# zhuye98/ICL

Measured on AMD Instinct MI355X. Metric: 3D volumes/sec/node (fwd+bwd, 96^3 patch), higher is better.
Workload: dtype f32; 1 GPU; 3D U-Net ICL BraTS-shape synthetic 96x96x96, num_classes=2, batch=2 per GPU (1 labeled + 1 unlabeled), full ICL step incl. SGD; global_batch=2, parallelism=dp1, launch=hipGraph replay

## Files before the change

### icl_amd/_lib.py

```python
from __future__ import annotations

import ctypes
import os
from ctypes import c_char_p, c_float, c_int, c_int64, c_void_p

import torch

_HERE = os.path.dirname(os.path.abspath(__file__))
DEFAULT_LIB = os.path.join(_HERE, "libicl_hip.so")

_lib = None
_lib_path = None
_host_pointers_ok = False

P, I, L, F = c_void_p, c_int, c_int64, c_float

_SIGNATURES = {
    "icl_abi_version": (c_int, []),
    "icl_last_error": (c_char_p, []),
    "icl_last_kernel_name": (c_char_p, []),
    "icl_conv3d_packed_elems": (c_int64, [I, I, I, I]),
    "icl_conv3d_pack_weights": (c_int, [P, P, I, I, I, I, P]),
    "icl_conv3d_pack_weights_both": (c_int, [P, P, P, I, I, I, P]),
    "icl_conv3d_pack_weights_multi": (c_int, [P, P, P, P, P, P, I, P]),
    "icl_conv3d_fwd_ws_bytes": (c_int64, [I, I, I, I, I, I, I]),
    "icl_conv3d_fwd": (c_int, [P, P, P, P, P, I, I, I, I, I, I, I, L, L, P]),
    "icl_scalar_combine": (c_int, [P, P, I, I, P, P]),
    "icl_conv3d_split_ws_bytes": (c_int64, [I, I]),
    "icl_conv3d_split_weights_multi": (c_int, [P, P, P, P, I, P]),
    "icl_conv3d_fwd_presplit": (c_int, [P, P, P, P, I, I, I, I, I, I, L, L, P]),
    "icl_conv3d_fwd_presplit_ws_bytes": (c_int64, [I, I, I, I, I, I]),
    "icl_conv3d_fwd_presplit_ws": (c_int, [P, P, P, P, P, I, I, I, I, I, I, L, L, P]),
    "icl_conv3d_fwd_stats_slots": (c_int, [I, I, I, I, I, I]),
    "icl_conv3d_fwd_presplit_stats": (c_int, [P, P, P, P, P, I, I, I, I, I, I, L, L, P]),
    "icl_norm_fwd_given_stats": (c_int, [P, P, P, P, P, P, P, P, P, I, I, L, I, I, F, F, P, I, P]),
    "icl_conv3d_wgrad_ws_bytes": (c_int64, [I, I, I, I]),
    "icl_conv3d_wgrad": (c_int, [P, P, P, P, P, I, I, I, I, I, I, I, L, L, P]),
    "icl_conv3d_wgrad_slabs": (c_int, [P, P, P, I, I, I, I, I, I, I, L, L, P, P]),
    "icl_conv3d_wgrad_reduce_multi": (c_int, [P, P, P, P, P, P, I, P]),
    "icl_norm_ws_bytes": (c_int64, [I, I, L]),
    "icl_norm_fwd": (c_int, [P, P, P, P, P, P, P, P, I, I, L, I, I, I, F, F, P, P]),
    "icl_norm_bwd": (c_int, [P, P, P, P, P, P, P, P, P, I, I, L, I, I, I, P, P]),
    "icl_norm_res_fwd": (c_int, [P, P, P, P, P, P, P, P, P, I, I, L, I, I, I, F, F, P, P]),
    "icl_norm_res_bwd": (c_int, [P, P, P, P, P, P, P, P, P, P, P, I, I, L, I, I, I, P, P]),
    "icl_rstd_from_var": (c_int, [P, P, I, F, P]),
    "icl_norm_finalize_stats": (c_int, [P, I, I, I, F, P, P, P, P]),
    "icl_norm_apply": (c_int, [P, P, P, I, I, L, P]),
    "icl_maxpool2_fwd_norm": (c_int, [P, P, P, P, L, I, I, I, I, P]),
    "icl_upsample2x_concat_norm": (c_int, [P, P, P, P, P, I, I, I, I, I, I, P]),
    "icl_conv1x1_dropout_norm": (c_int, [P, P, P, P, P, I, I, I, L, I, I, ctypes.c_uint32, F, P, P]),
    "icl_conv1x1_wgrad_dropout_norm": (c_int, [P, P, P, P, P, P, I, I, I, L, L, ctypes.c_uint32, F, P, P]),
    "icl_maxpool2_fwd": (c_int, [P, P, P, L, I, I, I, I, P]),
    "icl_maxpool2_bwd": (c_int, [P, P, P, L, I, I, I, I, P]),
    "icl_maxpool2_bwd_add": (c_int, [P, P, P, P, I, I, I, I, I, I, L, P]),
    "icl_trilinear_fwd": (c_int, [P, P, I, I, I, I, I, I, I, I, L, I, P]),
    "icl_trilinear_bwd_ws_bytes": (c_int64, [I, I, I, I, I, I, I, I]),
    "icl_trilinear_bwd": (c_int, [P, P, P, I, I, I, I, I, I, I, I, L, I, P]),
    "icl_copy_rows": (c_int, [P, P, L, L, L, L, P]),
    "icl_concat2": (c_int, [P, L, P, L, P, P]),
    "icl_dwconv3_fwd": (c_int, [P, P, P, I, I, I, I, I, I, P]),
    "icl_dwconv3_wgrad_ws_bytes": (c_int64, [I, I, I, I, I]),
    "icl_dwconv3_wgrad": (c_int, [P, P, P, P, I, I, I, I, I, P]),
    "icl_conv1x1_small": (c_int, [P, P, P, P, I, I, I, L, I, I, P]),
    "icl_conv1x1_dropout": (c_int, [P, P, P, P, I, I, I, L, I, I, I, ctypes.c_uint32, F, P, P]),
    "icl_conv1x1_wgrad_dropout": (c_int, [P, P, P, P, P, I, I, I, L, L, ctypes.c_uint32, F, P, P]),
    "icl_dropout": (c_int, [P, P, L, ctypes.c_uint32, F, P, P]),
    "icl_drop_path": (c_int, [P, P, L, L, ctypes.c_uint32, F, P, P]),
    "icl_drop_path_add": (c_int, [P, P, P, L, L, ctypes.c_uint32, F, P, P]),
    "icl_loss_fwd": (c_int, [P, P, P, P, P, P, I, I, L, I, I, P]),
    "icl_window_attn_bias_elems": (c_int64, [I, I]),
    "icl_depth_to_space2": (c_int, [P, P, I, I, I, I, I, L, P]),
    "icl_space_to_depth2": (c_int, [P, P, I, I, I, I, I, L, P]),
    "icl_colsum_multi": (c_int, [P, P, P, P, I, P]),
    "icl_gather_rows": (c_int, [P, P, P, L, L, L, I, P]),
    "icl_gather_rows_sum2": (c_int, [P, P, P, L, L, L, I, P]),
    "icl_im2col3": (c_int, [P, P, I, I, I, I, I, P]),
    "icl_im2col3_planes": (c_int, [P, P, I, I, I, I, I, P]),
    "icl_conv3d_cin1_fwd": (c_int, [P, P, P, P, I, I, I, I, I, L, L, P]),
    "icl_conv3d_cin1_wgrad_ws_bytes": (c_int64, [I, I, I]),
    "icl_conv3d_cin1_wgrad": (c_int, [P, P, P, P, I, I, I, I, I, L, L, P]),
    "icl_col2im3": (c_int, [P, P, I, I, I, I, I, P]),
    "icl_linear_ws_bytes": (c_int64, [L, I, I, I]),
    "icl_linear_fwd": (c_int, [P, P, P, P, P, L, I, I, I, P]),
    "icl_linear_dgrad": (c_int, [P, P, P, P, L, I, I, P]),
    "icl_linear_bwd_small": (c_int, [P, P, P, P, P, P, L, I, I, P]),
    "icl_linear_wgrad_small": (c_int, [P, P, P, P, L, I, I, P]),
    "icl_linear_dgrad_sgd": (c_int, [P, P, P, P, P, P, L, I, I, F, F, F, I, P, P]),
    "icl_gemm_ws_bytes": (c_int64, [L, I, I, I]),
    "icl_gemm": (c_int, [P, P, P, P, P, L, I, I, L, L, L, I, I, I, I, L, L, L, P]),
    "icl_linear_wgrad_ws_bytes": (c_int64, [L, I, I]),
    "icl_linear_wgrad": (c_int, [P, P, P, P, P, L, I, I, P]),
    "icl_conv1x1_wgrad_ws_bytes": (c_int64, [I, L, I, I]),
    "icl_conv1x1_wgrad": (c_int, [P, P, P, P, P, I, I, I, L, L, L, P]),
    "icl_relpos_bias_fwd": (c_int, [P, P, P, I, I, I, P]),
    "icl_window_attn_fwd": (c_int, [P, P, P, P, P, I, I, I, I, I, F, P]),
    "icl_window_attn_bwd": (c_int, [P, P, P, P, P, P, P, P, I, I, I, I, I, F, P]),
    "icl_window_attn_bwd_chunks": (c_int, [I, I, I, I, I]),
    "icl_relpos_bias_bwd_sum": (c_int, [P, I, P, P, P, L, I, I, P]),
    "icl_layernorm_fwd": (c_int, [P, P, P, P, P, P, L, I, F, P]),
    "icl_layernorm_bwd_ws_bytes": (c_int64, [L, I]),
    "icl_layernorm_bwd": (c_int, [P, P, P, P, P, P, P, P, P, L, I, P]),
    "icl_gelu_fwd": (c_int, [P, P, L, P]),
    "icl_gelu_bwd": (c_int, [P, P, P, L, P]),
    "icl_attn_fwd": (c_int, [P, P, P, P, P, I, I, I, I, I, F, P]),
    "icl_attn_bwd": (c_int, [P, P, P, P, P, P, P, P, P, I, I, I, I, I, F, P]),
    "icl_attn_bwd_ws_bytes": (c_int64, [I, I, I, I, I]),
    "icl_attn_bwd_ws": (c_int, [P, P, P, P, P, P, P, P, P, P, I, I, I, I, I, F, P]),
    "icl_crop_rotflip": (c_int, [P, P, P, I, P, P, I, I, I, P]),
    "icl_sgd_step": (c_int, [P, P, P, L, F, F, F, I, P, P]),
    "icl_sgd_step_factored": (c_int, [P, P, P, P, I, I, I, F, F, F, I, P, P]),
    "icl_sgd_step_factored_narrow": (c_int, [P, P, P, P, I, I, I, F, F, F, I, P, I, P]),
    "icl_sgd_factored_split_ws_bytes": (c_int64, [I, I, I]),
    "icl_sgd_step_factored_split": (c_int, [P, P, P, P, P, I, I, I, F, F, F, I, P, P]),
    "icl_sgd_step_multi": (c_int, [P, P, P, P, I, F, F, F, I, P, P]),
    "icl_loss_bwd": (c_int, [P, P, P, P, P, P, P, P, I, I, L, I, I, P]),
    "icl_loss_fwd_multi": (c_int, [P, I, P]),
    "icl_loss_bwd_multi": (c_int, [P, I, P]),
    "icl_qchain_stage": (c_int, [P, P]),
    "icl_qchain_wgrad": (c_int, [P, P, P, P, P, P, P, P, I, P]),
    "icl_seg_metrics_ws_bytes": (c_int64, [I, I, I, I]),
    "icl_seg_metrics": (c_int, [P, I, P, I, I, I, I, I, I, P, P, P]),
}

EXPORTS = tuple(_SIGNATURES)


def _load(path: str):
    if not os.path.exists(path):
        raise RuntimeError(
            f"icl_amd: HIP library {path} not found — build it with `python -m icl_amd.build` "
            "(hipcc --offload-arch=gfx950). There is no CPU fallback.")
    lib = ctypes.CDLL(path)
    for name, (res, args) in _SIGNATURES.items():
        fn = getattr(lib, name)
        fn.restype = res
        fn.argtypes = args
    return lib


def lib():
    global _lib, _lib_path
    if _lib is None:
        _lib_path = os.environ.get("ICL_HIP_LIB", DEFAULT_LIB)
        _lib = _load(_lib_path)
    return _lib


def lib_path():
    lib()
    return _lib_path


def host_pointers_ok() -> bool:
    return _host_pointers_ok


def _use_library_for_tests(path: str | None, host_pointers: bool = True):
    global _lib, _lib_path, _host_pointers_ok
    if path is None:
        _lib, _lib_path, _host_pointers_ok = None, None, False
        return
    _lib, _lib_path, _host_pointers_ok = _load(path), path, host_pointers


def check(rc: int, what: str = ""):
    if rc != 0:
        msg = lib().icl_last_error()
        raise RuntimeError(f"icl_hip {what} failed ({rc}): {msg.decode() if msg else ''}")
```

### icl_amd/csrc/icl_abi.inc

```

#include "kernels/common.h"
#include "kernels/norm.h"
#include "kernels/pool_resize.h"
#include "kernels/reduce.h"
#include "kernels/conv_mfma.h"
#include "kernels/conv_mfma_static.h"
#include "kernels/conv_mfma_flat.h"
#include "kernels/conv_bf16x3.h"
#include "kernels/conv_bf16x3_ws.h"
#include "kernels/conv_wgrad_tr.h"
#include "kernels/conv_wgrad_zs.h"
#include "kernels/conv_cin1.h"
#include "kernels/misc.h"
#include "kernels/loss.h"
#include "kernels/optim.h"
#include "kernels/winattn.h"
#include "kernels/linear_wgrad.h"
#include "kernels/token.h"
#include "kernels/gemm.h"
#include "kernels/datafeed.h"
#include "kernels/qchain.h"
#include "kernels/metrics.h"

#ifdef ICL_TWO_UNITS
// ... 992 lines not shown
int icl_conv3d_wgrad_slabs(const float* x, const float* gy, void* ws, int n, int cin, int cout, int d, int h, int w, int ks,
                           int64_t x_bstride, int64_t gy_bstride, int32_t* nslabs, void* stream) {
  if (!x || !gy || !ws || !nslabs || n < 1 || cin < 1 || cout < 1 || (ks != 1 && ks != 3)) return fail(-1, "conv3d_wgrad_slabs: bad argument");
  int ns = 0;
  const int rc = ks == 3 ? conv_wgrad_launch<3>(x, gy, (float*)ws, n, cin, cout, d, h, w, x_bstride, gy_bstride, &ns, (hipStream_t)stream)
                         : conv_wgrad_launch<1>(x, gy, (float*)ws, n, cin, cout, d, h, w, x_bstride, gy_bstride, &ns, (hipStream_t)stream);
  *nslabs = ns;
  return rc;
}

int icl_conv3d_wgrad_reduce_multi(const void* const* ws, void* const* gw, const int32_t* cout, const int32_t* cin, const int32_t* ks,
                                  const int32_t* nslabs, int count, void* stream) {
  if (!ws || !gw || !cout || !cin || !ks || !nslabs || count < 1) return fail(-1, "conv3d_wgrad_reduce_multi: bad argument");
  for (int base = 0; base < count; base += icl::kReduceMulti) {
    icl::ReduceMulti m{};
    const int k = count - base < icl::kReduceMulti ? count - base : icl::kReduceMulti;
    long most = 1;
    for (int i = 0; i < k; ++i) {
      const int j = base + i;
      if (!ws[j] || !gw[j] || cout[j] < 1 || cin[j] < 1 || (ks[j] != 1 && ks[j] != 3) || nslabs[j] < 1)
        return fail(-1, "conv3d_wgrad_reduce_multi: bad job %d", j);
      const long pe = icl_conv3d_packed_elems(cout[j], cin[j], ks[j], 0);
      m.gwp[i] = (const float*)ws[j]; m.gw[i] = (float*)gw[j];
      m.cout[i] = cout[j]; m.cin[i] = cin[j]; m.taps[i] = ks[j] * ks[j] * ks[j]; m.nslabs[i] = nslabs[j];
      m.tall[i] = wgrad_reduce_tall(nslabs[j], pe) ? 1 : 0;
      const long blocks = m.tall[i] ? cdivl(pe, 16) : cdivl(pe, 64);
      if (blocks > most) most = blocks;
    }
    ICL_LAUNCH(icl::reduce_unpack_wgrad_multi_kernel, dim3((unsigned)(most < 1024 ? most : 1024), k), dim3(256), 0, (hipStream_t)stream, m);
    const int rc = check_launch("reduce_unpack_wgrad_multi");
    if (rc) return rc;
  }
  return 0;
}

int icl_conv3d_wgrad(const float* x, const float* gy, float* gw, float* gbias, void* ws, int n, int cin, int cout, int d,
                     int h, int w, int ks, int64_t x_bstride, int64_t gy_bstride, void* stream) {
  if (!x || !gy || !gw || !ws || n < 1 || cin < 1 || cout < 1 || (ks != 1 && ks != 3)) return fail(-1, "conv3d_wgrad: bad argument");
  hipStream_t s = (hipStream_t)stream;
  float* gwp = (float*)ws;
  int nslabs = 0;
  int rc = ks == 3 ? conv_wgrad_launch<3>(x, gy, gwp, n, cin, cout, d, h, w, x_bstride, gy_bstride, &nslabs, s)
                   : conv_wgrad_launch<1>(x, gy, gwp, n, cin, cout, d, h, w, x_bstride, gy_bstride, &nslabs, s);
  if (rc) return rc;
  const int T = ks * ks * ks;
  const long total = (long)cout * cin * T;
  (void)total;
  const long pe_all = icl_conv3d_packed_elems(cout, cin, ks, 0);
  if (wgrad_reduce_tall(nslabs, pe_all))
    ICL_LAUNCH(icl::reduce_unpack_wgrad_tall_kernel, dim3((unsigned)cdivl(pe_all, 16)), dim3(256), 0, s, (const float*)gwp, gw, cout, cin, T,
               round_up(cin, 4), round_up(cout, 16), nslabs);
  else
    ICL_LAUNCH(icl::reduce_unpack_wgrad_kernel, dim3(grid_for(pe_all, 64)), dim3(256), 0, s, (const float*)gwp, gw, cout, cin, T,
               round_up(cin, 4), round_up(cout, 16), nslabs);
  rc = check_launch("reduce_unpack_wgrad");
  if (rc) return rc;
  if (gbias) {
    const long S = (long)d * h * w;
    long chunks = cdivl(S, 16384);
    if (chunks > 16) chunks = 16;
    const long clen = round_up(cdivl(S, chunks), 4);
    chunks = cdivl(S, clen);
    float* part = (float*)ws;
    dim3 grid((unsigned)chunks, cout, n);
    ICL_LAUNCH(icl::channel_sum_kernel, grid, dim3(256), 0, s, gy, part, S, (long)gy_bstride, clen);
    rc = check_launch("channel_sum");
    if (rc) return rc;
    const void* g[1] = {part};
    void* out[1] = {gbias};
    const int32_t rr[1] = {(int32_t)(n * chunks)}, cc[1] = {cout};
    rc = icl_colsum_multi(g, out, rr, cc, 1, stream);
  }
  return rc;
}

int64_t icl_norm_ws_bytes(int n, int c, int64_t s) {
  const int64_t nch = (s + icl::kNormChunk - 1) / icl::kNormChunk;
  return ((int64_t)n * c * nch * 3 + (int64_t)n * c * 2 + 64) * 4;
}

namespace {
inline bool norm_one_launch() {
  constexpr int on = 1;
  return on != 0;
}
}

int icl_norm_fwd(const float* x, float* y, float* mean, float* rstd, const float* gamma, const float* beta,
                 float* running_mean, float* running_var, int n, int c, int64_t s, int mode, int use_batch_stats,
                 int act, float eps, float momentum, void* ws, void* stream) {
  return icl_norm_res_fwd(x, nullptr, y, mean, rstd, gamma, beta, running_mean, running_var, n, c, s, mode, use_batch_stats, act,
                          eps, momentum, ws, stream);
}

int icl_norm_res_fwd(const float* x, const float* res, float* y, float* mean, float* rstd, const float* gamma, const float* beta,
                     float* running_mean, float* running_var, int n, int c, int64_t s, int mode, int use_batch_stats,
                     int act, float eps, float momentum, void* ws, void* stream) {
  if (!x || !y || !mean || !rstd || n < 1 || c < 1 || s < 1) return fail(-1, "norm_fwd: bad argument");
  hipStream_t st = (hipStream_t)stream;
  const int R = n * c;
  const int nch = (int)((s + icl::kNormChunk - 1) / icl::kNormChunk);
  const float* part = nullptr;
  const int inline_stats = (use_batch_stats && mode == 0 && nch == 1 && !running_mean && norm_one_launch()) ? 1 : 0;
  if (use_batch_stats && !inline_stats) {
    if (!ws) return fail(-1, "norm_fwd: workspace required");
    ICL_LAUNCH(icl::rowstats_partial_kernel, dim3(nch, R), dim3(icl::kNormThreads), 0, st, x, (float*)ws, (long)s, nch);
    if (int rc = check_launch("rowstats_partial")) return rc;
    part = (const float*)ws;
  }
  ICL_LAUNCH(icl::norm_act_fwd_kernel, dim3(nch, R), dim3(icl::kNormThreads), 0, st, x, y, mean, rstd, gamma, beta, (long)s, c, mode, act, res,
             part, R, nch, eps, running_mean, running_var, momentum, inline_stats);
  return check_launch("norm_act_fwd");
}

int icl_norm_fwd_given_stats(const float* x, const float* res, float* y, float* mean, float* rstd, const float* gamma, const float* beta,
                             float* running_mean, float* running_var, int n, int c, int64_t s, int mode, int act, float eps,
                             float momentum, const float* part, int nslots, void* stream) {
  if (!x || !y || !mean || !rstd || !part || n < 1 || c < 1 || s < 1 || nslots < 1) return fail(-1, "norm_fwd_given_stats: bad argument");
  const int R = n * c;
  const int nch = (int)((s + icl::kNormChunk - 1) / icl::kNormChunk);
  ICL_LAUNCH(icl::norm_act_fwd_kernel, dim3(nch, R), dim3(icl::kNormThreads), 0, (hipStream_t)stream, x, y, mean, rstd, gamma, beta, (long)s, c,
             mode, act, res, part, R, nslots, eps, running_mean, running_var, momentum, 0);
  return check_launch("norm_act_fwd");
}

int icl_norm_bwd(const float* gy, const float* x, const float* mean, const float* rstd, const float* gamma,
                 const float* beta, float* gx, float* dgamma, float* dbeta, int n, int c, int64_t s, int mode,
                 int use_batch_stats, int act, void* ws, void* stream) {
  return icl_norm_res_bwd(gy, x, nullptr, mean, rstd, gamma, beta, gx, nullptr, dgamma, dbeta, n, c, s, mode, use_batch_stats, act,
                          ws, stream);
}

int icl_norm_res_bwd(const float* gy, const float* x, const float* res, const float* mean, const float* rstd, const float* gamma,
                     const float* beta, float* gx, float* gres, float* dgamma, float* dbeta, int n, int c, int64_t s, int mode,
                     int use_batch_stats, int act, void* ws, void* stream) {
  if (!gy || !x || !mean || !rstd || !gx || !ws || n < 1 || c < 1 || s < 1) return fail(-1, "norm_bwd: bad argument");
  hipStream_t st = (hipStream_t)stream;
  const int R = n * c;
  const int nch = (int)((s + icl::kNormChunk - 1) / icl::kNormChunk);
  float* part = (float*)ws;
  if (mode == 0 && nch == 1 && norm_one_launch()) {
    part = nullptr;
  } else {
    ICL_LAUNCH(icl::norm_act_bwd_partial_kernel, dim3(nch, R), dim3(icl::kNormThreads), 0, st, gy, x, mean, rstd, gamma, beta, part,
               (long)s, c, nch, mode, act, res);
    if (int rc = check_launch("norm_bwd_partial")) return rc;
  }
  const float inv_count = 1.0f / (float)((mode ? (int64_t)n : 1) * s);
  ICL_LAUNCH(icl::norm_act_bwd_apply_kernel, dim3(nch, R), dim3(icl::kNormThreads), 0, st, gy, x, mean, rstd, gamma, beta,
             (const float*)part, gx, (long)s, c, mode, act, inv_count, use_batch_stats, res, gres, R, nch, dgamma, dbeta);
  return check_launch("norm_bwd_apply");
}

int icl_rstd_from_var(const float* var, float* rstd, int c, float eps, void* stream) {
  if (!var || !rstd || c < 1) return fail(-1, "rstd_from_var: bad argument");
  ICL_LAUNCH(icl::rstd_from_var_kernel, dim3((c + 63) / 64), dim3(64), 0, (hipStream_t)stream, var, rstd, c, eps);
  return check_launch("rstd_from_var");
}

namespace {
int maxpool2_fwd_run(const float* x, const float* ss, float* y, uint8_t* idx, int64_t nc, int dout, int hout, int wout, int pool_depth,
                     hipStream_t st, const char* what) {
  const long total = nc * dout * hout * wout;
  const char* e_x2 = getenv("ICL_MAXPOOL_BWD_X2");
  if ((wout & 1) == 0 && aligned16(x) && ((uintptr_t)y & 7) == 0 && (e_x2 ? atoi(e_x2) : 1)) {
    ICL_LAUNCH(icl::maxpool2_fwd_x2_kernel, dim3(grid_for(total / 2, 256)), dim3(256), 0, st, x, y, idx, (long)nc, dout, hout, wout, pool_depth, ss);
  } else {
    ICL_LAUNCH(icl::maxpool2_fwd_kernel, dim3(grid_for(total, 256)), dim3(256), 0, st, x, y, idx, (long)nc, dout, hout, wout, pool_depth, ss);
  }
  return check_launch(what);
}
}

int icl_maxpool2_fwd(const float* x, float* y, uint8_t* idx, int64_t nc, int dout, int hout, int wout, int pool_depth, void* stream) {
  if (!x || !y || !idx || nc < 1 || dout < 1 || hout < 1 || wout < 1 || (pool_depth != 1 && pool_depth != 2)) return fail(-1, "maxpool2_fwd: bad argument");
  return maxpool2_fwd_run(x, nullptr, y, idx, nc, dout, hout, wout, pool_depth, (hipStream_t)stream, "maxpool2_fwd");
}

int icl_norm_finalize_stats(const float* part, int n, int c, int nslots, float eps, float* mean, float* rstd, float* ss, void* stream) {
  if (!part || !mean || !rstd || !ss || n < 1 || c < 1 || nslots < 1) return fail(-1, "norm_finalize_stats: bad argument");
  ICL_LAUNCH(icl::norm_finalize_stats_kernel, dim3(n * c), dim3(64), 0, (hipStream_t)stream, part, n * c, c, nslots, eps, mean, rstd, ss);
  return check_launch("norm_finalize_stats");
}

int icl_norm_apply(const float* x, const float* ss, float* y, int n, int c, int64_t s, void* stream) {
  if (!x || !ss || !y || n < 1 || c < 1 || s < 4 || (s & 3) || !aligned16(x) || !aligned16(y)) return fail(-1, "norm_apply: bad argument (s %% 4 == 0)");
  ICL_LAUNCH(icl::copy_rows_norm_kernel, dim3(grid_for((long)n * c * (s >> 2), 256, 1 << 16)), dim3(256), 0, (hipStream_t)stream, x, y, n, c, (long)s,
             (long)c * s, ss);
  return check_launch("norm_apply");
}

int icl_maxpool2_fwd_norm(const float* x, const float* ss, float* y, uint8_t* idx, int64_t nc, int dout, int hout, int wout, int pool_depth,
                          void* stream) {
  if (!x || !ss || !y || !idx || nc < 1 || dout < 1 || hout < 1 || wout < 1 || (pool_depth != 1 && pool_depth != 2))
    return fail(-1, "maxpool2_fwd_norm: bad argument");
  return maxpool2_fwd_run(x, ss, y, idx, nc, dout, hout, wout, pool_depth, (hipStream_t)stream, "maxpool2_fwd_norm");
}

int icl_upsample2x_concat_norm(const float* skip, const float* skip_ss, const float* deep, const float* deep_ss, float* out, int n, int cs,
                               int cd, int d, int h, int w, void* stream) {
  if (!skip || !deep || !out || n < 1 || cs < 1 || cd < 1 || d < 2 || h < 2 || w < 4 || (d & 1) || (h & 1) || (w & 3))
    return fail(-1, "upsample2x_concat_norm: bad argument (even depth / height, width a multiple of 4)");
  if (!aligned16(skip) || !aligned16(deep) || !aligned16(out)) return fail(-1, "upsample2x_concat_norm: 16-byte alignment");
  hipStream_t st = (hipStream_t)stream;
  const long s = (long)d * h * w, obs = (long)(cs + cd) * s;
  if (skip_ss) {
    ICL_LAUNCH(icl::copy_rows_norm_kernel, dim3(grid_for((long)n * cs * (s >> 2), 256, 1 << 16)), dim3(256), 0, st, skip, out, n, cs, s, obs, skip_ss);
  } else {
    ICL_LAUNCH(icl::copy_rows_kernel, dim3(grid_for((long)n * cs * s, 256)), dim3(256), 0, st, skip, out, (long)n, (long)cs * s, (long)cs * s, obs);
  }
  if (int rc = check_launch("upsample2x_concat_norm: skip")) return rc;
  const long total = (long)n * cd * s;
  const int di = d / 2, hi = h / 2, wi = w / 2;
  if (wi % 4 == 0)
    ICL_LAUNCH(icl::upsample2x_fwd_x4_kernel, dim3(grid_for(total / 32, 256, 1 << 16)), dim3(256), 0, st, deep, out + (long)cs * s, n, cd, di, hi, wi, obs,
               deep_ss);
  else
    ICL_LAUNCH(icl::upsample2x_fwd_kernel, dim3(grid_for(total / 16, 256, 1 << 16)), dim3(256), 0, st, deep, out + (long)cs * s, n, cd, di, hi, wi, obs,
               deep_ss);
  return check_launch("upsample2x_concat_norm: deep");
}

int icl_maxpool2_bwd(const float* gy, const uint8_t* idx, float* gx, int64_t nc, int dout, int hout, int wout, int pool_depth, void* stream) {
  if (!gy || !gx || !idx || nc < 1 || dout < 1 || hout < 1 || wout < 1 || (pool_depth != 1 && pool_depth != 2)) return fail(-1, "maxpool2_bwd: bad argument");
  const long total = nc * dout * hout * wout;
  ICL_LAUNCH(icl::maxpool2_bwd_kernel, dim3(grid_for(total, 256)), dim3(256), 0, (hipStream_t)stream, gy, idx, gx, (long)nc, dout, hout, wout,
             pool_depth);
  return check_launch("maxpool2_bwd");
}

int icl_maxpool2_bwd_add(const float* gy, const uint8_t* idx, const float* add, float* gx, int n, int c, int dout, int hout, int wout,
                         int pool_depth, int64_t add_bstride, void* stream) {
  if (!gy || !gx || !idx || !add || n < 1 || c < 1 || dout < 1 || hout < 1 || wout < 1 || (pool_depth != 1 && pool_depth != 2) || (add_bstride & 1) ||
      ((uintptr_t)add & 7))
    return fail(-1, "maxpool2_bwd_add: bad argument");
  const long total = (long)n * c * dout * hout * wout;
  const char* e_x2 = getenv("ICL_MAXPOOL_BWD_X2");
  if ((wout & 1) == 0 && aligned16(add) && aligned16(gx) && ((uintptr_t)gy & 7) == 0 && (add_bstride & 3) == 0 && (e_x2 ? atoi(e_x2) : 1)) {
    ICL_LAUNCH(icl::maxpool2_bwd_add_x2_kernel, dim3(grid_for(total / 2, 256)), dim3(256), 0, (hipStream_t)stream, gy, idx, add, gx, (long)n * c, c,
               dout, hout, wout, pool_depth, (long)add_bstride);
    return check_launch("maxpool2_bwd_add_x2");
  }
  ICL_LAUNCH(icl::maxpool2_bwd_add_kernel, dim3(grid_for(total, 256)), dim3(256), 0, (hipStream_t)stream, gy, idx, add, gx, (long)n * c, c, dout,
             hout, wout, pool_depth, (long)add_bstride);
  return check_launch("maxpool2_bwd_add");
}

namespace {
inline float resize_scale(int in, int out, int align) {
  if (align) return out > 1 ? (float)(in - 1) / (float)(out - 1) : 0.f;
  return (float)in / (float)out;
}
}

int icl_trilinear_fwd(const float* x, float* y, int n, int c, int di, int hi, int wi, int dout, int hout, int wout,
                      int64_t y_bstride, int align_corners, void* stream) {
  if (!x || !y || n < 1 || c < 1 || di < 1 || hi < 1 || wi < 1 || dout < 1 || hout < 1 || wout < 1) return fail(-1, "trilinear_fwd: bad argument");
  const long total = (long)n * c * dout * hout * wout;
  const float rz = resize_scale(di, dout, align_corners), ry = resize_scale(hi, hout, align_corners), rx = resize_scale(wi, wout, align_corners);
  if (!align_corners && dout == 2 * di && hout == 2 * hi && wout == 2 * wi && wi % 2 == 0 && y_bstride % 4 == 0 && aligned16(y) &&
      total / 16 < (1L << 31)) {
    constexpr int x4 = 1;
    if (x4 && wi % 4 == 0 && aligned16(x))
      ICL_LAUNCH(icl::upsample2x_fwd_x4_kernel, dim3(grid_for(total / 32, 256, 1 << 16)), dim3(256), 0, (hipStream_t)stream, x, y, n, c, di, hi,
                 wi, (long)y_bstride, (const float*)nullptr);
    else
      ICL_LAUNCH(icl::upsample2x_fwd_kernel, dim3(grid_for(total / 16, 256, 1 << 16)), dim3(256), 0, (hipStream_t)stream, x, y, n, c, di, hi, wi,
                 (long)y_bstride, (const float*)nullptr);
  } else if (wout % 4 == 0 && y_bstride % 4 == 0 && aligned16(y) && total / 4 < (1L << 31)) {
    ICL_LAUNCH(icl::trilinear_fwd_quad_kernel, dim3(grid_for(total / 4, 256, 1 << 16)), dim3(256), 0, (hipStream_t)stream, x, y, n, c, di, hi,
               wi, dout, hout, wout, rz, ry, rx, (long)y_bstride, align_corners);
  } else {
    ICL_LAUNCH(icl::trilinear_fwd_kernel, dim3(grid_for(total, 256)), dim3(256), 0, (hipStream_t)stream, x, y, n, c, di, hi, wi, dout, hout,
               wout, rz, ry, rx, (long)y_bstride, align_corners);
  }
  return check_launch("trilinear_fwd");
}

int64_t icl_trilinear_bwd_ws_bytes(int n, int c, int di, int hi, int wi, int dout, int hout, int wout) {
  (void)di;
  return ((int64_t)n * c * dout * hout * wi + (int64_t)n * c * dout * hi * wi) * 4;
}

int icl_trilinear_bwd(const float* gy, float* gx, void* ws, int n, int c, int di, int hi, int wi, int dout, int hout, int wout,
                      int64_t gy_bstride, int align_corners, void* stream) {
  if (!gy || !gx || !ws || n < 1 || c < 1 || di < 1 || hi < 1 || wi < 1 || dout < 1 || hout < 1 || wout < 1) return fail(-1, "trilinear_bwd: bad argument");
  hipStream_t st = (hipStream_t)stream;
  const int al = align_corners;
  const float rz = resize_scale(di, dout, al), ry = resize_scale(hi, hout, al), rx = resize_scale(wi, wout, al);
  float* t1 = (float*)ws;
  float* t2 = t1 + (size_t)n * c * dout * hout * wi;
  int rc;
  if (!al && dout == 2 * di && hout == 2 * hi && wout == 2 * wi && wi % 4 == 0 && gy_bstride % 4 == 0 && aligned16(gy) && aligned16(gx) &&
      (long)n * c * di * hi * wi / 4 < (1L << 31)) {
    ICL_LAUNCH(icl::upsample2x_bwd_kernel, dim3(grid_for((long)n * c * ((di + icl::kUpSeg - 1) / icl::kUpSeg) * hi * wi / 4, 256, 1 << 16)),
               dim3(256), 0, st, gy, gx, n, c, di, hi,
               wi, (long)gy_bstride);
    return check_launch("upsample2x_bwd");
  }
  auto axis = [&](const float* src, float* dst, long rows, int li, int lo, long inner, float rs, long sbs, const char* what) -> int {
    const long total = (long)n * rows * li * inner;
    const bool small = total / 4 < (1L << 31) && rows < (1L << 31);
    if (small && inner % 4 == 0 && sbs % 4 == 0 && aligned16(src) && aligned16(dst)) {
      ICL_LAUNCH(icl::resize_bwd_axis_t4_kernel, dim3(grid_for(total / 4, 256, 1 << 16)), dim3(256), 0, st, src, dst, n, (unsigned)rows, li, lo,
                 (unsigned)(inner / 4), rs, sbs, al);
    } else if (inner == 1 && lo >= 4 * li && lo % 4 == 0 && lo <= 1024 && sbs % 4 == 0 && aligned16(src) && rows * li >= 4096) {
      const long nrows = (long)n * rows;
      ICL_LAUNCH(icl::resize_bwd_axis_x_lds_kernel, dim3((unsigned)cdivl(nrows, icl::kRbxRows)), dim3(256),
                 (size_t)icl::kRbxRows * (lo + 4) * 4, st, src, dst, n, rows, li, lo, rs, sbs, al);
    } else if (small && inner == 1 && li % 4 == 0 && aligned16(dst)) {
      ICL_LAUNCH(icl::resize_bwd_axis_i4_kernel, dim3(grid_for(total / 4, 256, 1 << 16)), dim3(256), 0, st, src, dst, n, (unsigned)rows, li, lo,
                 rs, sbs, al);
    } else {
      ICL_LAUNCH(icl::resize_bwd_axis_kernel, dim3(grid_for(total, 256)), dim3(256), 0, st, src, dst, n, rows, li, lo, inner, rs, sbs, al);
    }
    return check_launch(what);
  };
  if ((rc = axis(gy, t1, (long)c * dout * hout, wi, wout, 1L, rx, (long)gy_bstride, "resize_bwd_x"))) return rc;
  if ((rc = axis(t1, t2, (long)c * dout, hi, hout, (long)wi, ry, (long)c * dout * hout * wi, "resize_bwd_y"))) return rc;
  if ((rc = axis(t2, gx, (long)c, di, dout, (long)hi * wi, rz, (long)c * dout * hi * wi, "resize_bwd_z"))) return rc;
  return 0;
}

int icl_copy_rows(const float* src, float* dst, int64_t rows, int64_t row_elems, int64_t src_stride, int64_t dst_stride,
                  void* stream) {
  if (!src || !dst || rows < 1 || row_elems < 1) return fail(-1, "copy_rows: bad argument");
  ICL_LAUNCH(icl::copy_rows_kernel, dim3(grid_for(rows * row_elems, 256)), dim3(256), 0, (hipStream_t)stream, src, dst, (long)rows,
             (long)row_elems, (long)src_stride, (long)dst_stride);
  return check_launch("copy_rows");
}

int icl_concat2(const float* a, int64_t na, const float* b, int64_t nb, float* out, void* stream) {
  if (!out || na < 0 || nb < 0 || na + nb < 4 || (na & 3) || (nb & 3) || (!a && !b)) return fail(-1, "concat2: bad argument (float counts are multiples of 4)");
  if ((a && !aligned16(a)) || (b && !aligned16(b)) || !aligned16(out)) return fail(-1, "concat2: 16-byte alignment");
  ICL_LAUNCH(icl::concat2_kernel, dim3(grid_for((na + nb) >> 2, 256)), dim3(256), 0, (hipStream_t)stream, a, (long)na, b, (long)nb, out);
  return check_launch("concat2");
}

int icl_depth_to_space2(const float* yt, float* out, int n, int d, int h, int w, int cout, int64_t out_bstride, void* stream) {
  if (!yt || !out || n < 1 || d < 1 || h < 1 || w < 1 || cout < 1) return fail(-1, "depth_to_space2: bad argument");
  const size_t lds = (size_t)w * (cout * 8 + 2) * 4;
  if (lds > (size_t)kMaxDynLdsBig) return fail(-1, "depth_to_space2: token row does not fit LDS (w * cout too large)");
  if (lds > (size_t)kMaxDynLds) ICL_SET_MAX_DYN_LDS(icl::depth_to_space2_kernel, kMaxDynLdsBig);
  ICL_LAUNCH(icl::depth_to_space2_kernel, dim3(h, d, n), dim3(256), lds, (hipStream_t)stream, yt, out, d, h, w, cout, (long)out_bstride);
  return check_launch("depth_to_space2");
}

int icl_space_to_depth2(const float* g, float* gt, int n, int d, int h, int w, int cout, int64_t g_bstride, void* stream) {
  if (!g || !gt || n < 1 || d < 1 || h < 1 || w < 1 || cout < 1) return fail(-1, "space_to_depth2: bad argument");
  const size_t lds = (size_t)w * (cout * 8 + 2) * 4;
  if (lds > (size_t)kMaxDynLdsBig) return fail(-1, "space_to_depth2: token row does not fit LDS (w * cout too large)");
  if (lds > (size_t)kMaxDynLds) ICL_SET_MAX_DYN_LDS(icl::space_to_depth2_kernel, kMaxDynLdsBig);
  ICL_LAUNCH(icl::space_to_depth2_kernel, dim3(h, d, n), dim3(256), lds, (hipStream_t)stream, g, gt, d, h, w, cout, (long)g_bstride);
  return check_launch("space_to_depth2");
}

int icl_dwconv3_fwd(const float* x, const float* w, float* y, int n, int c, int d, int h, int wd, int flip, void* stream) {
  if (!x || !w || !y || n < 1 || c < 1 || d < 1 || h < 1 || wd < 1) return fail(-1, "dwconv3_fwd: bad argument");
  const long total = (long)n * c * d * h * wd;
  ICL_LAUNCH(icl::dwconv3_fwd_kernel, dim3(grid_for(total, 256)), dim3(256), 0, (hipStream_t)stream, x, w, y, (long)n * c, c, d, h, wd, flip);
  return check_launch("dwconv3_fwd");
}

static long dwconv3_wgrad_chunks(long total) {
  long chunks = cdivl(total, 1024);
  return chunks > 512 ? 512 : chunks;
}

int64_t icl_dwconv3_wgrad_ws_bytes(int n, int c, int d, int h, int wd) {
  return dwconv3_wgrad_chunks((long)n * d * h * wd) * c * 27 * 4;
}

int icl_dwconv3_wgrad(const float* x, const float* gy, float* gw, void* ws, int n, int c, int d, int h, int wd, void* stream) {
  if (!x || !gy || !gw || !ws || n < 1 || c < 1 || d < 1 || h < 1 || wd < 1) return fail(-1, "dwconv3_wgrad: bad argument");
  hipStream_t s = (hipStream_t)stream;
  const long total = (long)n * d * h * wd;
  const long chunks = dwconv3_wgrad_chunks(total);
  const long chunk = cdivl(total, chunks);
  ICL_LAUNCH(icl::dwconv3_wgrad_kernel, dim3((unsigned)chunks, c), dim3(256), 0, s, x, gy, (float*)ws, n, c, d, h, wd, chunk);
  if (int rc = check_launch("dwconv3_wgrad")) return rc;
  ICL_LAUNCH(icl::dwconv3_wgrad_reduce_kernel, dim3((unsigned)cdivl((long)c * 27, 16)), dim3(256), 0, s, (const float*)ws, gw, c * 27, (int)chunks);
  return check_launch("dwconv3_wgrad_reduce");
}

namespace {
icl::DropSpec drop_spec(int mode, uint32_t seed, float p, const uint32_t* seed_dev) {
  icl::DropSpec d{};
  d.mode = mode;
  d.seed = (unsigned)seed;
  d.thresh = (unsigned)((double)p * 4294967296.0);
  d.scale = 1.0f / (1.0f - p);
  d.seed_dev = (const unsigned*)seed_dev;
  return d;
}

int conv1x1_small_run(const float* x, const float* w, const float* bias, float* y, int n, int cin, int cout, int64_t s, int w_ostride,
                      int w_istride, const icl::DropSpec& dr, hipStream_t st) {
  if ((long)n * s >= 65536) {
// ... 278 lines not shown
  if (c >= 1024 && c <= 256 * 64 && longrow) {
    if (c <= 256 * 16) ICL_LAUNCH((icl::layernorm_bwd_longrow_kernel<16>), dim3((unsigned)rows), dim3(256), 0, st, gy, x, gamma, mean, rstd, gx, c);
    else if (c <= 256 * 32) ICL_LAUNCH((icl::layernorm_bwd_longrow_kernel<32>), dim3((unsigned)rows), dim3(256), 0, st, gy, x, gamma, mean, rstd, gx, c);
    else ICL_LAUNCH((icl::layernorm_bwd_longrow_kernel<64>), dim3((unsigned)rows), dim3(256), 0, st, gy, x, gamma, mean, rstd, gx, c);
  } else if (c >= 1024) {
    ICL_LAUNCH((icl::layernorm_bwd_kernel<true>), dim3((unsigned)rows), dim3(256), 0, st, gy, x, gamma, mean, rstd, gx, (long)rows, c);
  } else {
    ICL_LAUNCH((icl::layernorm_bwd_kernel<false>), dim3((unsigned)cdivl(rows, 4)), dim3(256), 0, st, gy, x, gamma, mean, rstd, gx,
               (long)rows, c);
  }
  int rc = check_launch("layernorm_bwd");
  if (rc || !ws) return rc;
  int cols = 256;
  while (cols > c && cols > 16) cols >>= 1;
  if (cols < c && cols < 256) cols <<= 1;
  ICL_LAUNCH(icl::layernorm_wgrad_kernel, dim3((c + cols - 1) / cols, (unsigned)chunks), dim3(256), 0, st, gy, x, mean, rstd, part_g, part_b,
             (long)rows, c, rpb, cols);
  rc = check_launch("layernorm_wgrad");
  if (rc || !dgamma) return rc;
  const void* g[2] = {part_g, part_b};
  void* out[2] = {dgamma, dbeta};
  const int32_t rr[2] = {chunks, chunks}, cc[2] = {c, c};
  return icl_colsum_multi(g, out, rr, cc, 2, stream);
}

int icl_gelu_fwd(const float* x, float* y, int64_t n, void* stream) {
  if (!x || !y || n < 1) return fail(-1, "gelu_fwd: bad argument");
  ICL_LAUNCH(icl::gelu_fwd_kernel, dim3(grid_for(n, 256)), dim3(256), 0, (hipStream_t)stream, x, y, (long)n);
  return check_launch("gelu_fwd");
}

int icl_gelu_bwd(const float* gy, const float* x, float* gx, int64_t n, void* stream) {
  if (!gy || !x || !gx || n < 1) return fail(-1, "gelu_bwd: bad argument");
  ICL_LAUNCH(icl::gelu_bwd_kernel, dim3(grid_for(n, 256)), dim3(256), 0, (hipStream_t)stream, gy, x, gx, (long)n);
  return check_launch("gelu_bwd");
}

int icl_attn_fwd(const float* q, const float* kv, float* logits, float* out, float* stats, int b, int h, int nc, int n, int d,
                 float scale, void* stream) {
  if (!q || !kv || !logits || !out || !stats || b < 1 || h < 1 || nc < 1 || nc > icl::kAttnMaxNc || n < 1 || (d != 8 && d != 16))
    return fail(-1, "attn_fwd: bad argument (nc <= 16, head dim 8 or 16)");
  hipStream_t st = (hipStream_t)stream;
  const dim3 g1((n + 255) / 256, b * h), g2(b * h * nc);
  if (d == 16) {
    ICL_LAUNCH((icl::attn_logits_kernel<16>), g1, dim3(256), 0, st, q, kv, logits, b, h, nc, n, scale);
    ICL_LAUNCH((icl::attn_softmax_pv_kernel<16, 256>), g2, dim3(256), 0, st, (const float*)logits, kv, out, stats, b, h, nc, n);
  } else {
    ICL_LAUNCH((icl::attn_logits_kernel<8>), g1, dim3(256), 0, st, q, kv, logits, b, h, nc, n, scale);
    ICL_LAUNCH((icl::attn_softmax_pv_kernel<8, 256>), g2, dim3(256), 0, st, (const float*)logits, kv, out, stats, b, h, nc, n);
  }
  return check_launch("attn_fwd");
}

int64_t icl_attn_bwd_ws_bytes(int b, int h, int nc, int n, int d) {
  if (b < 1 || h < 1 || nc < 1 || n < 1 || d < 1) return 0;
  return (int64_t)((n + 255) / 256) * b * h * nc * d * 4;
}

int icl_attn_bwd(const float* q, const float* kv, const float* logits, const float* stats, const float* out, const float* gout,
                 const float* glog, float* gq, float* gkv, int b, int h, int nc, int n, int d, float scale, void* stream) {
  return icl_attn_bwd_ws(q, kv, logits, stats, out, gout, glog, gq, gkv, nullptr, b, h, nc, n, d, scale, stream);
}

int icl_attn_bwd_ws(const float* q, const float* kv, const float* logits, const float* stats, const float* out, const float* gout,
                    const float* glog, float* gq, float* gkv, void* ws, int b, int h, int nc, int n, int d, float scale, void* stream) {
  if (!q || !kv || !logits || !stats || !out || !gq || !gkv || b < 1 || h < 1 || nc < 1 || nc > icl::kAttnMaxNc || n < 1 ||
      (d != 8 && d != 16))
    return fail(-1, "attn_bwd: bad argument");
  hipStream_t st = (hipStream_t)stream;
  const dim3 g1((n + 255) / 256, b * h), g2(b * h * nc);
  float* pq = (float*)ws;
  if (d == 16) {
    ICL_LAUNCH((icl::attn_bwd_kv_kernel<16>), g1, dim3(256), 0, st, q, kv, logits, stats, out, gout, glog, gkv, b, h, nc, n, scale, pq);
    if (!pq) ICL_LAUNCH((icl::attn_bwd_q_kernel<16, 256>), g2, dim3(256), 0, st, kv, logits, stats, out, gout, glog, gq, b, h, nc, n, scale);
  } else {
    ICL_LAUNCH((icl::attn_bwd_kv_kernel<8>), g1, dim3(256), 0, st, q, kv, logits, stats, out, gout, glog, gkv, b, h, nc, n, scale, pq);
    if (!pq) ICL_LAUNCH((icl::attn_bwd_q_kernel<8, 256>), g2, dim3(256), 0, st, kv, logits, stats, out, gout, glog, gq, b, h, nc, n, scale);
  }
  if (pq) {
    const int rd = b * h * nc * d;
    ICL_LAUNCH(icl::attn_dq_reduce_kernel, dim3((rd + 255) / 256), dim3(256), 0, st, (const float*)pq, gq, (int)g1.x, rd, scale);
  }
  return check_launch("attn_bwd");
}

int64_t icl_window_attn_bias_elems(int n, int heads) { return icl_window_attn_bias_elems_impl(n, heads); }

static int linear_wgrad_nsplit(int64_t rows, int o, int i) {
  const int ob = (o + icl::kLwB - 1) / icl::kLwB, ib = (i + icl::kLwB - 1) / icl::kLwB;
  long n = rows * (o + i) / ((long)o * i + o);
  const long want = (2048 + ob * ib - 1) / (ob * ib);
  if (n > want) n = want;
  const long steps = (rows + 3) / 4;
  if (n > steps / 8) n = steps / 8;
  if (n < 4) n = 4;
  return (int)((n + 3) / 4 * 4);
}

int64_t icl_linear_wgrad_ws_bytes(int64_t rows, int o, int i) {
  return (int64_t)linear_wgrad_nsplit(rows, o, i) * ((int64_t)o * i + o) * 4;
}

int icl_linear_wgrad(const float* gy, const float* x, float* dw, float* db, void* ws, int64_t rows, int o, int i, void* stream) {
  if (!gy || !x || !dw || !ws || rows < 1 || o < 1 || i < 1) return fail(-1, "linear_wgrad: bad argument");
  hipStream_t st = (hipStream_t)stream;
  const int nsplit = linear_wgrad_nsplit(rows, o, i);
  const int ob = (o + icl::kLwB - 1) / icl::kLwB, ib = (i + icl::kLwB - 1) / icl::kLwB;
  ICL_LAUNCH(icl::linear_wgrad_kernel, dim3(nsplit / 4, ob, ib), dim3(256), 0, st, gy, x, (float*)ws, (long)rows, o, i, nsplit);
  if (int rc = check_launch("linear_wgrad")) return rc;
  const long EW = (long)o * i, E = EW + o;
  ICL_LAUNCH(icl::linear_wgrad_reduce_kernel, dim3((unsigned)cdivl(E, 16)), dim3(256), 0, st, (const float*)ws, dw, db, E, EW, nsplit);
  return check_launch("linear_wgrad_reduce");
}

static bool cin1_geom(icl::Cin1Geom& g, int n, int cout, int d, int h, int w, int64_t xbs, int64_t ybs) {
  if (n < 1 || cout < 1 || cout > 16 || d < 1 || h < 1 || w < 1 || (long)d * h * w * 16 >= (1L << 31)) return false;
  g.N = n; g.Cout = cout; g.D = d; g.H = h; g.W = w; g.nty = (h + icl::kC1Rows - 1) / icl::kC1Rows;
  g.x_bstride = xbs; g.y_bstride = ybs; g.ntiles = n * d * g.nty;
  return (size_t)3 * (icl::kC1Rows + 2) * (w + 2) * 4 <= 64 * 1024;
}
static int cin1_grid(const icl::Cin1Geom& g) { return g.ntiles < 2048 ? g.ntiles : 2048; }
static size_t cin1_lds(const icl::Cin1Geom& g) {
  const size_t halo = (size_t)3 * (icl::kC1Rows + 2) * (g.W + 2) * 4;
  return halo > 2048 * 4 ? halo : 2048 * 4;
}

int icl_conv3d_cin1_fwd(const float* x, const float* w, const float* bias, float* y, int n, int cout, int d, int h, int wd, int64_t x_bstride,
                        int64_t y_bstride, void* stream) {
  icl::Cin1Geom g;
  if (!x || !w || !y || !cin1_geom(g, n, cout, d, h, wd, x_bstride, y_bstride)) return fail(-1, "conv3d_cin1_fwd: bad argument");
  ICL_LAUNCH(icl::conv_cin1_fwd_kernel, dim3(cin1_grid(g)), dim3(icl::kC1Threads), cin1_lds(g), (hipStream_t)stream, x, w, bias, y, g);
  snprintf(g_kernel, sizeof(g_kernel), "conv_cin1_fwd_kernel");
  return check_launch("conv3d_cin1_fwd");
}

int64_t icl_conv3d_cin1_wgrad_ws_bytes(int n, int d, int h) {
  const long tiles = (long)n * d * ((h + icl::kC1Rows - 1) / icl::kC1Rows);
  return (tiles < 2048 ? tiles : 2048) * 512 * 4;
}

int icl_conv3d_cin1_wgrad(const float* x, const float* gy, float* gw, void* ws, int n, int cout, int d, int h, int wd, int64_t x_bstride,
                          int64_t gy_bstride, void* stream) {
  icl::Cin1Geom g;
  if (!x || !gy || !gw || !ws || (wd & 3) || (gy_bstride & 3) || !aligned16(gy) || !cin1_geom(g, n, cout, d, h, wd, x_bstride, gy_bstride))
    return fail(-1, "conv3d_cin1_wgrad: bad argument (W and the sample stride of dY must be multiples of 4, dY 16-byte aligned)");
  const int grid = cin1_grid(g);
  ICL_LAUNCH(icl::conv_cin1_wgrad_kernel, dim3(grid), dim3(icl::kC1Threads), cin1_lds(g), (hipStream_t)stream, x, gy, (float*)ws, g);
  if (int rc = check_launch("conv3d_cin1_wgrad")) return rc;
  ICL_LAUNCH(icl::conv_cin1_wgrad_reduce_kernel, dim3(16), dim3(256), 0, (hipStream_t)stream, (const float*)ws, gw, grid, cout);
  snprintf(g_kernel, sizeof(g_kernel), "conv_cin1_wgrad_kernel");
  return check_launch("conv3d_cin1_wgrad_reduce");
}

int64_t icl_conv1x1_wgrad_ws_bytes(int n, int64_t s, int cin, int cout) { return icl_linear_wgrad_ws_bytes((int64_t)n * s, cout, cin); }

namespace {
int conv1x1_wgrad_run(const float* x, const float* gy, float* gw, float* gbias, void* ws, int n, int cin, int cout, int64_t s,
                      int64_t x_bstride, int64_t gy_bstride, const icl::DropSpec& dr, hipStream_t st) {
  const int nsplit = linear_wgrad_nsplit((int64_t)n * s, cout, cin);
  const int ob = (cout + icl::kLwB - 1) / icl::kLwB, ib = (cin + icl::kLwB - 1) / icl::kLwB;
  ICL_LAUNCH(icl::conv1x1_wgrad_kernel, dim3(nsplit / 4, ob, ib), dim3(256), 0, st, gy, x, (float*)ws, n, (long)s, cout, cin, nsplit,
             (long)gy_bstride, (long)x_bstride, dr);
  if (int rc = check_launch("conv1x1_wgrad")) return rc;
  const long EW = (long)cout * cin, E = EW + cout;
  ICL_LAUNCH(icl::linear_wgrad_reduce_kernel, dim3((unsigned)cdivl(E, 16)), dim3(256), 0, st, (const float*)ws, gw, gbias, E, EW, nsplit);
  return check_launch("conv1x1_wgrad_reduce");
}
}

int icl_conv1x1_wgrad(const float* x, const float* gy, float* gw, float* gbias, void* ws, int n, int cin, int cout, int64_t s,
                      int64_t x_bstride, int64_t gy_bstride, void* stream) {
  if (!x || !gy || !gw || !ws || n < 1 || cin < 1 || cout < 1 || s < 4 || (s & 3) || (x_bstride & 3) || (gy_bstride & 3))
    return fail(-1, "conv1x1_wgrad: bad argument (voxel count and batch strides must be multiples of 4)");
  return conv1x1_wgrad_run(x, gy, gw, gbias, ws, n, cin, cout, s, x_bstride, gy_bstride, icl::DropSpec{}, (hipStream_t)stream);
}

int icl_conv1x1_wgrad_dropout(const float* x, const float* gy, float* gw, float* gbias, void* ws, int n, int cin, int cout, int64_t s,
                              int64_t gy_bstride, uint32_t seed, float p, const uint32_t* seed_dev, void* stream) {
  if (!x || !gy || !gw || !ws || n < 1 || cin < 1 || cout < 1 || s < 4 || (s & 3) || (gy_bstride & 3) || !(p >= 0.f && p < 1.f))
    return fail(-1, "conv1x1_wgrad_dropout: bad argument");
  return conv1x1_wgrad_run(x, gy, gw, gbias, ws, n, cin, cout, s, (int64_t)cin * s, gy_bstride, drop_spec(1, seed, p, seed_dev), (hipStream_t)stream);
}

int icl_conv1x1_wgrad_dropout_norm(const float* x, const float* ss, const float* gy, float* gw, float* gbias, void* ws, int n, int cin, int cout,
                                   int64_t s, int64_t gy_bstride, uint32_t seed, float p, const uint32_t* seed_dev, void* stream) {
  if (!x || !ss || !gy || !gw || !ws || n < 1 || cin < 1 || cout < 1 || s < 4 || (s & 3) || (gy_bstride & 3) || !(p >= 0.f && p < 1.f))
    return fail(-1, "conv1x1_wgrad_dropout_norm: bad argument");
  icl::DropSpec dr = p > 0.f ? drop_spec(1, seed, p, seed_dev) : icl::DropSpec{};
  dr.ss = ss;
  return conv1x1_wgrad_run(x, gy, gw, gbias, ws, n, cin, cout, s, (int64_t)cin * s, gy_bstride, dr, (hipStream_t)stream);
}

int icl_relpos_bias_fwd(const float* table, const int64_t* index, float* bias, int n, int heads, int idx_stride, void* stream) {
  if (!table || !index || !bias || n < 1 || n > idx_stride || heads < 1) return fail(-1, "relpos_bias_fwd: bad argument");
  const int npad = (n + 15) / 16 * 16;
  ICL_LAUNCH(icl::relpos_bias_gather_kernel, dim3(grid_for((long)heads * n * npad, 256)), dim3(256), 0, (hipStream_t)stream, table,
             (const long*)index, bias, n, npad, heads, idx_stride);
  return check_launch("relpos_bias_fwd");
}

int icl_window_attn_fwd(const float* qkv, const float* bias, const int32_t* regions, float* out, float* lse, int b_, int n, int heads,
                        int nw, int head_dim, float scale, void* stream) {
  if (!qkv || !bias || !out || !lse) return fail(-1, "window_attn_fwd: null pointer");
  icl::WinAttnGeom g;
  if (int rc = winattn_geom(g, b_, n, heads, nw, head_dim, scale, "window_attn_fwd")) return rc;
  const int nkb = g.npad / 16;
  hipStream_t st = (hipStream_t)stream;
  const char* e_on = getenv("ICL_WINATTN_ONLINE");
  const int online = e_on ? atoi(e_on) : 1;
  if (head_dim == 16 && ((nkb > 6 && (long)g.B_ * g.heads >= 512 && online == 1) || online == 2)) {
    const size_t lds = ((size_t)2 * g.npad * (16 + 4) + g.npad) * 4;
    ICL_SET_MAX_DYN_LDS((icl::window_attn_fwd_online_kernel<16>), 64 * 1024);
    ICL_LAUNCH((icl::window_attn_fwd_online_kernel<16>), dim3((unsigned)g.B_ * g.heads), dim3(icl::kWaThreads), lds, st, qkv, bias, regions,
               out, lse, g);
    snprintf(g_kernel, sizeof(g_kernel), "window_attn_fwd_online_kernel<16>");
    return check_launch("window_attn_fwd_online");
  }
  if (head_dim == 32) return winattn_fwd_launch<6, 32>(qkv, bias, regions, out, lse, g, st);
  if (nkb > 14) return winattn_fwd_launch<22, 16>(qkv, bias, regions, out, lse, g, st);
  if (nkb > 6) return winattn_fwd_launch<14, 16>(qkv, bias, regions, out, lse, g, st);
  return winattn_fwd_launch<6, 16>(qkv, bias, regions, out, lse, g, st);
}

int icl_window_attn_bwd(const float* qkv, const float* bias, const int32_t* regions, const float* out, const float* lse,
                        const float* dout, float* dqkv, float* dbias, int b_, int n, int heads, int nw, int head_dim, float scale,
                        void* stream) {
  if (!qkv || !bias || !out || !lse || !dout || !dqkv) return fail(-1, "window_attn_bwd: null pointer");
  icl::WinAttnGeom g;
  if (int rc = winattn_geom(g, b_, n, heads, nw, head_dim, scale, "window_attn_bwd")) return rc;
  hipStream_t st = (hipStream_t)stream;
  if (int rc = head_dim == 32 ? winattn_kv_launch<32>(qkv, bias, regions, out, lse, dout, dqkv, g, st)
                              : winattn_kv_launch<16>(qkv, bias, regions, out, lse, dout, dqkv, g, st))
    return rc;
  const int nkb = g.npad / 16;
  if (head_dim == 32) return winattn_q_bias_launch<6, 32>(qkv, bias, regions, out, lse, dout, dqkv, dbias, g, st);
  if (nkb > 14) return winattn_q_bias_launch<22, 16>(qkv, bias, regions, out, lse, dout, dqkv, dbias, g, st);
  if (nkb > 6) return winattn_q_bias_launch<14, 16>(qkv, bias, regions, out, lse, dout, dqkv, dbias, g, st);
  return winattn_q_bias_launch<6, 16>(qkv, bias, regions, out, lse, dout, dqkv, dbias, g, st);
}

int icl_window_attn_bwd_chunks(int b_, int n, int heads, int nw, int head_dim) {
  icl::WinAttnGeom g;
  if (winattn_geom(g, b_, n, heads, nw, head_dim, 1.f, "window_attn_bwd_chunks")) return 0;
  return winattn_bias_chunks(g);
}

int icl_relpos_bias_bwd_sum(float* dbias, int chunks, const int32_t* inv, const int32_t* offs, float* dtable, int64_t table_rows, int n,
                            int heads, void* stream) {
  if (!dbias || !inv || !offs || !dtable || chunks < 1 || n < 1 || heads < 1 || table_rows < 1)
    return fail(-1, "relpos_bias_bwd_sum: bad argument");
  const int npad = (n + 15) / 16 * 16;
  if (chunks > 1) {
    const long slab = (long)heads * n * npad;
    ICL_LAUNCH(icl::relpos_bias_slab_sum_kernel, dim3(grid_for(slab / 4, 256, 1024)), dim3(256), 0, (hipStream_t)stream, dbias,
               slab, chunks);
    if (int rc = check_launch("relpos_bias_slab_sum")) return rc;
  }
  ICL_LAUNCH(icl::relpos_bias_gather_sum_kernel, dim3((unsigned)((table_rows + 3) / 4), heads), dim3(256), 0, (hipStream_t)stream, dbias, inv,
             offs, dtable, (int)table_rows, n, npad, heads, 1);
  return check_launch("relpos_bias_bwd_sum");
}

int icl_sgd_step(float* p, const float* g, float* m, int64_t n, float lr, float momentum, float weight_decay, int first,
                 const float* lr_dev, void* stream) {
  if (!p || !g || !m || n < 1) return fail(-1, "sgd_step: bad argument");
  ICL_LAUNCH(icl::sgd_momentum_kernel, dim3(grid_for((n + 3) / 4, 256, 4096)), dim3(256), 0, (hipStream_t)stream, p, g, m, (long)n, lr,
             momentum, weight_decay, first, lr_dev);
  return check_launch("sgd_step");
}

int64_t icl_sgd_factored_split_ws_bytes(int rows, int n, int k) {
  if (rows < 1 || n < 1 || k < 1) return 0;
  return (int64_t)3 * ((rows + 7) / 8) * ((int64_t)n + k) * 16;
}

int icl_sgd_step_factored_split(float* p, float* m, const float* g, const float* x, void* ws, int rows, int n, int k, float lr,
                                float momentum, float weight_decay, int first, const float* lr_dev, void* stream) {
  if (!p || !m || !g || !x || !ws || rows < 1 || n < 1 || k < 4 || (k & 3) || !aligned16(ws))
    return fail(-1, "sgd_step_factored_split: bad argument (k %% 4 == 0, workspace of icl_sgd_factored_split_ws_bytes)");
  hipStream_t st = (hipStream_t)stream;
  const int mb = (rows + 7) / 8;
  uint4* gs = (uint4*)ws;
  uint4* xs = gs + (size_t)3 * mb * n;
  ICL_LAUNCH(icl::factor_split_kernel, dim3(grid_for((long)mb * ((long)n + k), 256, 2048)), dim3(256), 0, st, g, x, gs, xs, rows, n, k);
  int rc = check_launch("factor_split");
  if (rc) return rc;
  const size_t lds = (size_t)icl::kSfLdsFloats * 4;
  ICL_SET_MAX_DYN_LDS(icl::sgd_factored_split_kernel, kMaxDynLdsBig);
  ICL_LAUNCH(icl::sgd_factored_split_kernel, dim3((k + icl::kSfCols - 1) / icl::kSfCols, (n + icl::kSfRows - 1) / icl::kSfRows), dim3(256), lds,
             st, p, m, (const uint4*)gs, (const uint4*)xs, rows, n, k, lr, momentum, weight_decay, first, lr_dev);
  return check_launch("sgd_step_factored_split");
}

int icl_sgd_step_factored(float* p, float* m, const float* g, const float* x, int rows, int n, int k, float lr, float momentum,
                          float weight_decay, int first, const float* lr_dev, void* stream) {
  if (!p || !m || !g || !x || rows < 1 || n < 1 || k < 4 || (k & 3)) return fail(-1, "sgd_step_factored: bad argument (k %% 4 == 0)");
  if (rows <= 16) {
    constexpr int variant = 2;
    const dim3 grid((k + icl::kSvCols - 1) / icl::kSvCols, (n + icl::kSvRows - 1) / icl::kSvRows);
    if (variant == 2) {
      ICL_LAUNCH(icl::sgd_factored_small_kernel<2>, grid, dim3(256), 0, (hipStream_t)stream, p, m, g, x, rows, n, k, lr, momentum, weight_decay,
                 first, lr_dev);
    } else if (variant == 1) {
      ICL_LAUNCH(icl::sgd_factored_small_kernel<1>, grid, dim3(256), 0, (hipStream_t)stream, p, m, g, x, rows, n, k, lr, momentum, weight_decay,
                 first, lr_dev);
    } else {
// ... 317 lines not shown
```

### icl_amd/csrc/kernels/conv_cin1.h

```cpp
#pragma once

namespace icl {

constexpr int kC1Rows = 8, kC1Threads = 256;

struct Cin1Geom {
  int N, Cout, D, H, W, nty;
  long x_bstride, y_bstride;
  int ntiles;
};

__device__ __forceinline__ void c1_stage_halo(float* xs, const float* __restrict__ x, const Cin1Geom& g, int n, int z, int y0) {
  const int PW = g.W + 2, PR = kC1Rows + 2;
  const long HW = (long)g.H * g.W;
  const float* xb = x + (long)n * g.x_bstride;
  for (int it = threadIdx.x; it < 3 * PR * PW; it += kC1Threads) {
    const int px = it % PW, row = it / PW, py = row % PR, pz = row / PR;
    const int gz = z - 1 + pz, gy = y0 - 1 + py, gx = px - 1;
    float v = 0.f;
    if ((unsigned)gz < (unsigned)g.D && (unsigned)gy < (unsigned)g.H && (unsigned)gx < (unsigned)g.W) v = xb[gz * HW + (long)gy * g.W + gx];
    xs[it] = v;
  }
}

__global__ __launch_bounds__(kC1Threads) void conv_cin1_wgrad_kernel(const float* __restrict__ x, const float* __restrict__ gy,
                                                                     float* __restrict__ part, Cin1Geom g) {
  ICL_DYN_LDS(float, xs);
  const int lane = threadIdx.x & 63, wid = threadIdx.x >> 6, lr = lane & 15, lg = lane >> 4;
  const int PW = g.W + 2, PR = kC1Rows + 2;
  const long HW = (long)g.H * g.W, DHW = g.D * HW;
  int toff[2];
  bool tok[2];
#pragma unroll
  for (int tb = 0; tb < 2; ++tb) {
    const int tap = 16 * tb + lr;
    tok[tb] = tap < 27;
    const int t = tok[tb] ? tap : 0;
    toff[tb] = (t / 9) * PR * PW + ((t / 3) % 3) * PW + t % 3;
  }
  f32x4 acc[2] = {f32x4{0.f, 0.f, 0.f, 0.f}, f32x4{0.f, 0.f, 0.f, 0.f}};
  for (int tile = blockIdx.x; tile < g.ntiles; tile += gridDim.x) {
    const int n = tile / (g.D * g.nty), rem = tile % (g.D * g.nty), z = rem / g.nty, y0 = (rem % g.nty) * kC1Rows;
    __syncthreads();
    c1_stage_halo(xs, x, g, n, z, y0);
    __syncthreads();
    const float* gb = gy + (long)n * g.y_bstride + (long)lr * DHW + (long)z * HW;
    for (int rr = 0; rr < 2; ++rr) {
      const int ty = 2 * wid + rr, yy = y0 + ty;
      if (yy >= g.H) break;
      const float* grow = gb + (long)yy * g.W;
      const float* xrow = xs + (ty * PW);
      for (int x0 = 0; x0 < g.W; x0 += 16) {
        const int xl = x0 + 4 * lg;
        float4 a = make_float4(0.f, 0.f, 0.f, 0.f);
        if (lr < g.Cout && xl < g.W) a = *reinterpret_cast<const float4*>(grow + xl);
        const float av[4] = {a.x, a.y, a.z, a.w};
        const bool in = xl < g.W;
#pragma unroll
        for (int j = 0; j < 4; ++j) {
#pragma unroll
          for (int tb = 0; tb < 2; ++tb) {
            const float b = (tok[tb] && in) ? xrow[toff[tb] + xl + j] : 0.f;
            acc[tb] = icl_mfma_16x16x4(av[j], b, acc[tb]);
          }
        }
      }
    }
  }
  __syncthreads();
  float* red = xs;
#pragma unroll
  for (int tb = 0; tb < 2; ++tb)
#pragma unroll
    for (int r = 0; r < 4; ++r) red[((wid * 2 + tb) * 4 + r) * 64 + lane] = acc[tb][r];
  __syncthreads();
  if (wid == 0) {
#pragma unroll
    for (int tb = 0; tb < 2; ++tb)
#pragma unroll
      for (int r = 0; r < 4; ++r) {
        float s = 0.f;
#pragma unroll
        for (int w = 0; w < 4; ++w) s += red[((w * 2 + tb) * 4 + r) * 64 + lane];
        part[(long)blockIdx.x * 512 + (4 * lg + r) * 32 + 16 * tb + lr] = s;
      }
  }
}

__global__ __launch_bounds__(256) void conv_cin1_wgrad_reduce_kernel(const float* __restrict__ part, float* __restrict__ gw, int nparts, int cout) {
  __shared__ float sl[8][32];
  const int o = threadIdx.x & 31, slice = threadIdx.x >> 5, e = blockIdx.x * 32 + o;
  float s = 0.f;
#pragma unroll 8
  for (int p = slice; p < nparts; p += 8) s += part[(long)p * 512 + e];
  sl[slice][o] = s;
  __syncthreads();
  if (slice == 0) {
    float t = 0.f;
#pragma unroll
    for (int k = 0; k < 8; ++k) t += sl[k][o];
    const int co = e >> 5, tap = e & 31;
    if (co < cout && tap < 27) gw[co * 27 + tap] = t;
  }
}

__global__ __launch_bounds__(kC1Threads) void conv_cin1_fwd_kernel(const float* __restrict__ x, const float* __restrict__ w,
                                                                   const float* __restrict__ bias, float* __restrict__ y, Cin1Geom g) {
  ICL_DYN_LDS(float, xs);
  const int lane = threadIdx.x & 63, wid = threadIdx.x >> 6, lr = lane & 15, lg = lane >> 4;
  const int PW = g.W + 2, PR = kC1Rows + 2;
  const long HW = (long)g.H * g.W, DHW = g.D * HW;
  float wa[7];
  int toff[7];
#pragma unroll
  for (int s = 0; s < 7; ++s) {
    const int tap = 4 * s + lg;
    wa[s] = (tap < 27 && lr < g.Cout) ? w[lr * 27 + tap] : 0.f;
    const int t = tap < 27 ? tap : 0;
    toff[s] = (t / 9) * PR * PW + ((t / 3) % 3) * PW + t % 3;
  }
  float bv[4];
#pragma unroll
  for (int r = 0; r < 4; ++r) bv[r] = (bias && 4 * lg + r < g.Cout) ? bias[4 * lg + r] : 0.f;
  for (int tile = blockIdx.x; tile < g.ntiles; tile += gridDim.x) {
    const int n = tile / (g.D * g.nty), rem = tile % (g.D * g.nty), z = rem / g.nty, y0 = (rem % g.nty) * kC1Rows;
    __syncthreads();
    c1_stage_halo(xs, x, g, n, z, y0);
    __syncthreads();
    float* yb = y + (long)n * g.y_bstride + (long)z * HW;
    for (int rr = 0; rr < 2; ++rr) {
      const int ty = 2 * wid + rr, yy = y0 + ty;
      if (yy >= g.H) break;
      const float* xrow = xs + ty * PW;
      for (int x0 = 0; x0 < g.W; x0 += 16) {
        const int xp = x0 + lr;
        const bool in = xp < g.W;
        f32x4 acc = f32x4{bv[0], bv[1], bv[2], bv[3]};
#pragma unroll
        for (int s = 0; s < 7; ++s) acc = icl_mfma_16x16x4(wa[s], in ? xrow[toff[s] + xp] : 0.f, acc);
        if (in) {
#pragma unroll
          for (int r = 0; r < 4; ++r)
            if (4 * lg + r < g.Cout) yb[(long)(4 * lg + r) * DHW + (long)yy * g.W + xp] = acc[r];
        }
      }
    }
  }
}

}
```

### icl_amd/csrc/kernels/norm.h

```cpp
#pragma once

namespace icl {

constexpr int kNormChunk = 8192;
constexpr int kNormThreads = 256;

__device__ __forceinline__ void row_chunk_summary(const float* __restrict__ xr, long lo, long hi, long S, float& tn, float& tm, float& tq) {
  float n = 0.f, shift = 0.f, s1 = 0.f, s2 = 0.f;
  if ((S & 3) == 0) {
    const float4* x4 = reinterpret_cast<const float4*>(xr);
#pragma unroll 4
    for (long i = (lo >> 2) + threadIdx.x; i < (hi >> 2); i += kNormThreads) {
      const float4 v = x4[i];
      if (n == 0.f) shift = v.x;
      const float d0 = v.x - shift, d1 = v.y - shift, d2 = v.z - shift, d3 = v.w - shift;
      float a1 = d0 + d1, b1 = d2 + d3, a2 = d0 * d0 + d1 * d1, b2 = d2 * d2 + d3 * d3;
      ICL_PIN1(a1); ICL_PIN1(b1); ICL_PIN1(a2); ICL_PIN1(b2);
      s1 += a1 + b1;
      s2 += a2 + b2;
      n += 4.f;
    }
  } else {
    for (long i = lo + threadIdx.x; i < hi; i += kNormThreads) {
      const float v = xr[i];
// ... 50 lines not shown
__device__ __forceinline__ void norm_group_stats(const float* __restrict__ part, int g, int R, int C, int nchunks, int batch_mode,
                                                 float& mean_out, float& var_out, float& n_out) {
  __shared__ float bc[3];
  if (threadIdx.x < 64) {
    const int lane = threadIdx.x;
    float n = 0.f, m = 0.f, q = 0.f;
    const int step = batch_mode ? C : R;
    const int nrows = (R - g + step - 1) / step;
    const long items = (long)nrows * nchunks;
    for (long it = lane; it < items; it += 64) {
      const int r = g + (int)(it / nchunks) * step;
      const float* p = part + ((long)r * nchunks + it % nchunks) * 3;
      welford_merge(n, m, q, p[0], p[1], p[2]);
    }
#pragma unroll
    for (int sh = 32; sh >= 1; sh >>= 1) {
      const float nb = __shfl_xor(n, sh, 64), mb = __shfl_xor(m, sh, 64), qb = __shfl_xor(q, sh, 64);
      welford_merge(n, m, q, nb, mb, qb);
    }
    if (lane == 0) { bc[0] = m; bc[1] = q / n; bc[2] = n; }
  }
  __syncthreads();
  mean_out = bc[0]; var_out = bc[1]; n_out = bc[2];
}

__global__ __launch_bounds__(64) void norm_finalize_stats_kernel(const float* __restrict__ part, int R, int C, int nchunks, float eps,
                                                                 float* __restrict__ mean, float* __restrict__ rstd, float* __restrict__ ss) {
  const int g = blockIdx.x;
  float m, var, n;
  norm_group_stats(part, g, R, C, nchunks, 0, m, var, n);
  if (threadIdx.x == 0) {
    const float rs = 1.0f / sqrtf(var + eps);
    mean[g] = m;
    rstd[g] = rs;
    ss[2 * g] = rs;
    ss[2 * g + 1] = 0.f - m * rs;
  }
}

__global__ __launch_bounds__(kNormThreads) void norm_act_fwd_kernel(
    const float* __restrict__ x, float* __restrict__ y, float* __restrict__ mean,
    float* __restrict__ rstd, const float* __restrict__ gamma, const float* __restrict__ beta,
    long S, int C, int batch_mode, int act, const float* __restrict__ res, const float* __restrict__ part, int R, int nchunks,
    float eps, float* running_mean, float* running_var, float momentum, int inline_stats) {
  const long r = blockIdx.y;
  const int c = (int)(r % C);
  const int g = batch_mode ? c : (int)r;
  float m, rs;
  if (part == nullptr && inline_stats) {
    __shared__ float bcs[2];
    float tn, tm, tq;
    row_chunk_summary(x + r * S, 0, S, S, tn, tm, tq);
    if (threadIdx.x == 0) { bcs[0] = tm; bcs[1] = tq / tn; }
    __syncthreads();
    m = bcs[0];
    rs = 1.0f / sqrtf(bcs[1] + eps);
    if (threadIdx.x == 0) { mean[g] = m; rstd[g] = rs; }
  } else if (part) {
    float var, n;
    norm_group_stats(part, g, R, C, nchunks, batch_mode, m, var, n);
    rs = 1.0f / sqrtf(var + eps);
    if (threadIdx.x == 0 && blockIdx.x == 0 && (!batch_mode || r < C)) {
      mean[g] = m;
      rstd[g] = rs;
      if (running_mean) {
        const float unbiased = n > 1.f ? var * n / (n - 1.f) : var;
        running_mean[g] = (1.f - momentum) * running_mean[g] + momentum * m;
        running_var[g] = (1.f - momentum) * running_var[g] + momentum * unbiased;
      }
    }
  } else {
    m = mean[g];
    rs = rstd[g];
  }
  const float ga = gamma ? gamma[c] : 1.f, be = beta ? beta[c] : 0.f;
  const float sc = rs * ga, sh = be - m * rs * ga;
  const long lo = (long)blockIdx.x * kNormChunk;
  const long hi = (lo + kNormChunk < S) ? lo + kNormChunk : S;
  const float* xr = x + r * S;
  float* yr = y + r * S;
  const float* rr = res ? res + r * S : nullptr;
  if ((S & 3) == 0) {
    const float4* x4 = reinterpret_cast<const float4*>(xr);
    const float4* r4 = reinterpret_cast<const float4*>(rr);
    float4* y4 = reinterpret_cast<float4*>(yr);
#pragma unroll 4
    for (long i = (lo >> 2) + threadIdx.x; i < (hi >> 2); i += kNormThreads) {
      float4 v = x4[i];
      v.x = v.x * sc + sh; v.y = v.y * sc + sh; v.z = v.z * sc + sh; v.w = v.w * sc + sh;
      if (rr) { const float4 q = r4[i]; v.x += q.x; v.y += q.y; v.z += q.z; v.w += q.w; }
      if (act == 1) { v.x = fmaxf(v.x, 0.f); v.y = fmaxf(v.y, 0.f); v.z = fmaxf(v.z, 0.f); v.w = fmaxf(v.w, 0.f); }
      else if (act == 2) { v.x = v.x > 0.f ? v.x : 0.01f * v.x; v.y = v.y > 0.f ? v.y : 0.01f * v.y; v.z = v.z > 0.f ? v.z : 0.01f * v.z; v.w = v.w > 0.f ? v.w : 0.01f * v.w; }
      y4[i] = v;
    }
  } else {
    for (long i = lo + threadIdx.x; i < hi; i += kNormThreads) {
      float v = xr[i] * sc + sh;
      if (rr) v += rr[i];
      yr[i] = act == 1 ? fmaxf(v, 0.f) : (act == 2 && v < 0.f ? 0.01f * v : v);
    }
  }
}

__device__ __forceinline__ void norm_bwd_chunk_sums(const float* __restrict__ xr, const float* __restrict__ gr, const float* __restrict__ rr, long lo,
                                                    long hi, long S, float m, float rs, float ga, float be, int act, float& p1, float& p2) {
  p1 = 0.f; p2 = 0.f;
  if ((S & 3) == 0) {
    const float4* x4 = reinterpret_cast<const float4*>(xr);
    const float4* g4 = reinterpret_cast<const float4*>(gr);
    const float4* r4 = reinterpret_cast<const float4*>(rr);
#pragma unroll 4
    for (long i = (lo >> 2) + threadIdx.x; i < (hi >> 2); i += kNormThreads) {
      const float4 xv = x4[i], gv = g4[i];
      const float4 rv = rr ? r4[i] : make_float4(0.f, 0.f, 0.f, 0.f);
      const float xs[4] = {xv.x, xv.y, xv.z, xv.w}, gs[4] = {gv.x, gv.y, gv.z, gv.w}, rs4[4] = {rv.x, rv.y, rv.z, rv.w};
#pragma unroll
      for (int k = 0; k < 4; ++k) {
        const float xh = (xs[k] - m) * rs;
        float h = gs[k];
        if (act && !(xh * ga + be + rs4[k] > 0.f)) h = (act == 2) ? 0.01f * h : 0.f;
        p1 += h;
        p2 += h * xh;
      }
    }
  } else {
    for (long i = lo + threadIdx.x; i < hi; i += kNormThreads) {
      const float xh = (xr[i] - m) * rs;
      float h = gr[i];
      if (act && !(xh * ga + be + (rr ? rr[i] : 0.f) > 0.f)) h = (act == 2) ? 0.01f * h : 0.f;
      p1 += h;
      p2 += h * xh;
    }
  }
  __shared__ float red[kNormThreads / 64];
  p1 = block_sum<kNormThreads>(p1, red);
  p2 = block_sum<kNormThreads>(p2, red);
}

__global__ __launch_bounds__(kNormThreads) void norm_act_bwd_partial_kernel(
    const float* __restrict__ gy, const float* __restrict__ x, const float* __restrict__ mean,
    const float* __restrict__ rstd, const float* __restrict__ gamma, const float* __restrict__ beta,
    float* __restrict__ part, long S, int C, int nchunks, int batch_mode, int act, const float* __restrict__ res) {
  const long r = blockIdx.y;
  const int c = (int)(r % C);
  const int g = batch_mode ? c : (int)r;
  const long lo = (long)blockIdx.x * kNormChunk;
  const long hi = (lo + kNormChunk < S) ? lo + kNormChunk : S;
  float p1, p2;
  norm_bwd_chunk_sums(x + r * S, gy + r * S, res ? res + r * S : nullptr, lo, hi, S, mean[g], rstd[g], gamma ? gamma[c] : 1.f, beta ? beta[c] : 0.f,
                      act, p1, p2);
  if (threadIdx.x == 0) {
    float* p = part + (r * nchunks + blockIdx.x) * 2;
    p[0] = p1; p[1] = p2;
  }
}

__global__ __launch_bounds__(kNormThreads) void norm_act_bwd_apply_kernel(
    const float* __restrict__ gy, const float* __restrict__ x, const float* __restrict__ mean,
    const float* __restrict__ rstd, const float* __restrict__ gamma, const float* __restrict__ beta,
    const float* __restrict__ part, float* __restrict__ gx, long S, int C, int batch_mode, int act,
    float inv_count, int use_batch_stats, const float* __restrict__ res, float* __restrict__ gres, int R, int nchunks,
    float* __restrict__ dgamma, float* __restrict__ dbeta) {
  const long r = blockIdx.y;
  const int c = (int)(r % C);
  const int g = batch_mode ? c : (int)r;
  __shared__ float bc[2];
  if (part == nullptr) {
    float p1, p2;
    norm_bwd_chunk_sums(x + r * S, gy + r * S, res ? res + r * S : nullptr, 0, S, S, mean[g], rstd[g], gamma ? gamma[c] : 1.f,
                        beta ? beta[c] : 0.f, act, p1, p2);
    if (threadIdx.x == 0) { bc[0] = p1; bc[1] = p2; }
  } else if (threadIdx.x < 64) {
    const int lane = threadIdx.x;
    const int step = batch_mode ? C : R;
    const int nrows = (R - g + step - 1) / step;
    const long items = (long)nrows * nchunks;
    float p1 = 0.f, p2 = 0.f;
    for (long it = lane; it < items; it += 64) {
      const int rr_ = g + (int)(it / nchunks) * step;
      const float* p = part + ((long)rr_ * nchunks + it % nchunks) * 2;
      p1 += p[0];
      p2 += p[1];
    }
    p1 = wave_sum(p1);
    p2 = wave_sum(p2);
    if (lane == 0) { bc[0] = p1; bc[1] = p2; }
  }
  __syncthreads();
  const float P1 = bc[0], P2 = bc[1];
  if (batch_mode && dgamma && threadIdx.x == 0 && blockIdx.x == 0 && r < C) { dgamma[g] = P2; dbeta[g] = P1; }
  const float m = mean[g], rs = rstd[g];
  const float ga = gamma ? gamma[c] : 1.f, be = beta ? beta[c] : 0.f;
  const float a1 = use_batch_stats ? P1 * inv_count : 0.f;
  const float a2 = use_batch_stats ? P2 * inv_count : 0.f;
  const float k = rs * ga;
  const long lo = (long)blockIdx.x * kNormChunk;
  const long hi = (lo + kNormChunk < S) ? lo + kNormChunk : S;
  const float* xr = x + r * S;
  const float* gr = gy + r * S;
  float* o = gx + r * S;
  const float* rr = res ? res + r * S : nullptr;
  float* go = gres ? gres + r * S : nullptr;
  if ((S & 3) == 0) {
    const float4* x4 = reinterpret_cast<const float4*>(xr);
    const float4* g4 = reinterpret_cast<const float4*>(gr);
    const float4* r4 = reinterpret_cast<const float4*>(rr);
    float4* o4 = reinterpret_cast<float4*>(o);
    float4* go4 = reinterpret_cast<float4*>(go);
#pragma unroll 4
    for (long i = (lo >> 2) + threadIdx.x; i < (hi >> 2); i += kNormThreads) {
      const float4 xv = x4[i], gv = g4[i];
      const float4 rv = rr ? r4[i] : make_float4(0.f, 0.f, 0.f, 0.f);
      const float xs[4] = {xv.x, xv.y, xv.z, xv.w}, gs[4] = {gv.x, gv.y, gv.z, gv.w}, rs4[4] = {rv.x, rv.y, rv.z, rv.w};
      float ov[4], hv[4];
#pragma unroll
      for (int q = 0; q < 4; ++q) {
        const float xh = (xs[q] - m) * rs;
        float h = gs[q];
        if (act && !(xh * ga + be + rs4[q] > 0.f)) h = (act == 2) ? 0.01f * h : 0.f;
        ov[q] = k * (h - a1 - xh * a2);
        hv[q] = h;
      }
      o4[i] = make_float4(ov[0], ov[1], ov[2], ov[3]);
      if (go) go4[i] = make_float4(hv[0], hv[1], hv[2], hv[3]);
    }
    return;
  }
  for (long i = lo + threadIdx.x; i < hi; i += kNormThreads) {
    const float xh = (xr[i] - m) * rs;
    float h = gr[i];
    if (act && !(xh * ga + be + (rr ? rr[i] : 0.f) > 0.f)) h = (act == 2) ? 0.01f * h : 0.f;
    o[i] = k * (h - a1 - xh * a2);
    if (go) go[i] = h;
  }
}

}
```

### icl_amd/csrc/kernels/pool_resize.h

```cpp
#pragma once

namespace icl {

__global__ __launch_bounds__(256) void maxpool2_fwd_kernel(const float* __restrict__ x, float* __restrict__ y,
                                                           unsigned char* __restrict__ idx, long NC, int Do, int Ho, int Wo, int pd,
                                                           const float* __restrict__ ss) {
  const long total = NC * Do * Ho * Wo;
  const int H = Ho * 2, W = Wo * 2;
  const int nk = 4 * pd;
  for (long o = (long)blockIdx.x * blockDim.x + threadIdx.x; o < total; o += (long)gridDim.x * blockDim.x) {
    const int ox = (int)(o % Wo);
    long t = o / Wo;
    const int oy = (int)(t % Ho);
    t /= Ho;
    const int oz = (int)(t % Do);
    const long nc = t / Do;
    const float* p = x + ((nc * (Do * pd) + oz * pd) * H + oy * 2) * (long)W + ox * 2;
    const float sc = ss ? ss[2 * nc] : 1.f, sh = ss ? ss[2 * nc + 1] : 0.f;
    float best = ss ? norm_relu1(p[0], sc, sh) : p[0];
    int bi = 0;
    for (int k = 1; k < nk; ++k) {
      float v = p[((k >> 2) * H + ((k >> 1) & 1)) * (long)W + (k & 1)];
      if (ss) v = norm_relu1(v, sc, sh);
      if (v > best) { best = v; bi = k; }
    }
    y[o] = best;
    idx[o] = (unsigned char)bi;
  }
}

__global__ __launch_bounds__(256) void maxpool2_fwd_x2_kernel(const float* __restrict__ x, float* __restrict__ y,
                                                              unsigned char* __restrict__ idx, long NC, int Do, int Ho, int Wo, int pd,
                                                              const float* __restrict__ ss) {
  const int Wo2 = Wo >> 1;
  const long total = NC * Do * Ho * Wo2;
  const int H = Ho * 2, W = Wo * 2;
  const int nk = 4 * pd;
  for (long o2 = (long)blockIdx.x * blockDim.x + threadIdx.x; o2 < total; o2 += (long)gridDim.x * blockDim.x) {
    const int ox = (int)(o2 % Wo2) * 2;
    long t = o2 / Wo2;
    const int oy = (int)(t % Ho);
    t /= Ho;
    const int oz = (int)(t % Do);
    const long nc = t / Do;
    const long o = ((nc * Do + oz) * Ho + oy) * (long)Wo + ox;
    const float* p = x + ((nc * (Do * pd) + oz * pd) * H + oy * 2) * (long)W + ox * 2;
    const float sc = ss ? ss[2 * nc] : 1.f, sh = ss ? ss[2 * nc + 1] : 0.f;
    float b0 = 0.f, b1 = 0.f;
    int i0 = 0, i1 = 0;
    for (int k = 0; k < nk; k += 2) {
      float4 v = *reinterpret_cast<const float4*>(p + ((k >> 2) * H + ((k >> 1) & 1)) * (long)W);
      if (ss) { v.x = norm_relu1(v.x, sc, sh); v.y = norm_relu1(v.y, sc, sh); v.z = norm_relu1(v.z, sc, sh); v.w = norm_relu1(v.w, sc, sh); }
      if (k == 0) { b0 = v.x; b1 = v.z; }
      else {
        if (v.x > b0) { b0 = v.x; i0 = k; }
        if (v.z > b1) { b1 = v.z; i1 = k; }
      }
      if (v.y > b0) { b0 = v.y; i0 = k + 1; }
      if (v.w > b1) { b1 = v.w; i1 = k + 1; }
    }
    *reinterpret_cast<float2*>(y + o) = make_float2(b0, b1);
    idx[o] = (unsigned char)i0;
    idx[o + 1] = (unsigned char)i1;
  }
}

__global__ __launch_bounds__(256) void maxpool2_bwd_kernel(const float* __restrict__ gy, const unsigned char* __restrict__ idx,
                                                           float* __restrict__ gx, long NC, int Do, int Ho, int Wo, int pd) {
  const long total = NC * Do * Ho * Wo;
  const int H = Ho * 2, W = Wo * 2;
  const int nk = 4 * pd;
  for (long o = (long)blockIdx.x * blockDim.x + threadIdx.x; o < total; o += (long)gridDim.x * blockDim.x) {
    const int ox = (int)(o % Wo);
    long t = o / Wo;
    const int oy = (int)(t % Ho);
    t /= Ho;
    const int oz = (int)(t % Do);
    const long nc = t / Do;
    float* p = gx + ((nc * (Do * pd) + oz * pd) * H + oy * 2) * (long)W + ox * 2;
    const float g = gy[o];
    const int bi = idx[o];
    for (int k = 0; k < nk; k += 2) {
      float2 v = make_float2(bi == k ? g : 0.f, bi == k + 1 ? g : 0.f);
      *reinterpret_cast<float2*>(p + ((k >> 2) * H + ((k >> 1) & 1)) * (long)W) = v;
    }
  }
}

__global__ __launch_bounds__(256) void maxpool2_bwd_add_kernel(const float* __restrict__ gy, const unsigned char* __restrict__ idx,
                                                               const float* __restrict__ add, float* __restrict__ gx, long NC, int C, int Do,
                                                               int Ho, int Wo, int pd, long add_bstride) {
  const long total = NC * Do * Ho * Wo;
  const int H = Ho * 2, W = Wo * 2;
  const long plane = (long)Do * pd * H * W;
  const int nk = 4 * pd;
  for (long o = (long)blockIdx.x * blockDim.x + threadIdx.x; o < total; o += (long)gridDim.x * blockDim.x) {
    const int ox = (int)(o % Wo);
    long t = o / Wo;
    const int oy = (int)(t % Ho);
    t /= Ho;
    const int oz = (int)(t % Do);
    const long nc = t / Do;
    const long in_plane = ((long)(oz * pd) * H + oy * 2) * (long)W + ox * 2;
    float* p = gx + nc * plane + in_plane;
    const float* a = add + (nc / C) * add_bstride + (nc % C) * plane + in_plane;
    const float g = gy[o];
    const int bi = idx[o];
    for (int k = 0; k < nk; k += 2) {
      const long off = ((k >> 2) * H + ((k >> 1) & 1)) * (long)W;
      const float2 s = *reinterpret_cast<const float2*>(a + off);
      *reinterpret_cast<float2*>(p + off) = make_float2(s.x + (bi == k ? g : 0.f), s.y + (bi == k + 1 ? g : 0.f));
    }
  }
}

__global__ __launch_bounds__(256) void maxpool2_bwd_add_x2_kernel(const float* __restrict__ gy, const unsigned char* __restrict__ idx,
                                                                  const float* __restrict__ add, float* __restrict__ gx, long NC, int C, int Do,
                                                                  int Ho, int Wo, int pd, long add_bstride) {
  const int Wo2 = Wo >> 1;
  const long total = NC * Do * Ho * Wo2;
  const int H = Ho * 2, W = Wo * 2;
  const long plane = (long)Do * pd * H * W;
  const int nk = 4 * pd;
  for (long o2 = (long)blockIdx.x * blockDim.x + threadIdx.x; o2 < total; o2 += (long)gridDim.x * blockDim.x) {
    const int ox = (int)(o2 % Wo2) * 2;
    long t = o2 / Wo2;
    const int oy = (int)(t % Ho);
    t /= Ho;
    const int oz = (int)(t % Do);
    const long nc = t / Do;
    const long o = ((nc * Do + oz) * Ho + oy) * (long)Wo + ox;
    const long in_plane = ((long)(oz * pd) * H + oy * 2) * (long)W + ox * 2;
    float* p = gx + nc * plane + in_plane;
    const float* a = add + (nc / C) * add_bstride + (nc % C) * plane + in_plane;
    const float2 g = *reinterpret_cast<const float2*>(gy + o);
    const int b0 = idx[o], b1 = idx[o + 1];
    for (int k = 0; k < nk; k += 2) {
      const long off = ((k >> 2) * H + ((k >> 1) & 1)) * (long)W;
      const float4 s = *reinterpret_cast<const float4*>(a + off);
      *reinterpret_cast<float4*>(p + off) = make_float4(s.x + (b0 == k ? g.x : 0.f), s.y + (b0 == k + 1 ? g.x : 0.f),
                                                        s.z + (b1 == k ? g.y : 0.f), s.w + (b1 == k + 1 ? g.y : 0.f));
    }
  }
}

struct LinTap { int i0, i1; float l0, l1; };
__device__ __forceinline__ LinTap lin_tap(int dst, float rscale, int in_size, int align) {
  float src = align ? rscale * (float)dst : rscale * ((float)dst + 0.5f) - 0.5f;
  if (src < 0.f) src = 0.f;
  LinTap t;
  t.i0 = (int)src;
  if (t.i0 > in_size - 1) t.i0 = in_size - 1;
  t.i1 = t.i0 + (t.i0 < in_size - 1 ? 1 : 0);
  t.l1 = src - (float)t.i0;
  t.l0 = 1.f - t.l1;
  return t;
}

__global__ __launch_bounds__(256) void trilinear_fwd_kernel(const float* __restrict__ x, float* __restrict__ y, int N, int C,
                                                            int Di, int Hi, int Wi, int Do, int Ho, int Wo,
                                                            float rz, float ry, float rx, long y_bstride, int align) {
  const long per_n = (long)C * Do * Ho * Wo;
  const long total = (long)N * per_n;
  for (long o = (long)blockIdx.x * blockDim.x + threadIdx.x; o < total; o += (long)gridDim.x * blockDim.x) {
    const int ox = (int)(o % Wo);
    long t = o / Wo;
    const int oy = (int)(t % Ho);
    t /= Ho;
    const int oz = (int)(t % Do);
    t /= Do;
    const int c = (int)(t % C);
    const int n = (int)(t / C);
    const LinTap tz = lin_tap(oz, rz, Di, align), ty = lin_tap(oy, ry, Hi, align), tx = lin_tap(ox, rx, Wi, align);
    const float* p = x + ((long)n * C + c) * Di * Hi * Wi;
    const long z0 = (long)tz.i0 * Hi * Wi, z1 = (long)tz.i1 * Hi * Wi;
    const long y0 = (long)ty.i0 * Wi, y1 = (long)ty.i1 * Wi;
    const float v =
        tz.l0 * (ty.l0 * (tx.l0 * p[z0 + y0 + tx.i0] + tx.l1 * p[z0 + y0 + tx.i1]) +
                 ty.l1 * (tx.l0 * p[z0 + y1 + tx.i0] + tx.l1 * p[z0 + y1 + tx.i1])) +
        tz.l1 * (ty.l0 * (tx.l0 * p[z1 + y0 + tx.i0] + tx.l1 * p[z1 + y0 + tx.i1]) +
                 ty.l1 * (tx.l0 * p[z1 + y1 + tx.i0] + tx.l1 * p[z1 + y1 + tx.i1]));
    y[(long)n * y_bstride + (((long)c * Do + oz) * Ho + oy) * Wo + ox] = v;
  }
}

__global__ __launch_bounds__(256) void trilinear_fwd_quad_kernel(const float* __restrict__ x, float* __restrict__ y, int N, int C,
                                                                 int Di, int Hi, int Wi, int Do, int Ho, int Wo,
                                                                 float rz, float ry, float rx, long y_bstride, int align) {
  const unsigned wq = (unsigned)Wo >> 2;
  const unsigned total = (unsigned)N * C * Do * Ho * wq;
  for (unsigned e = blockIdx.x * blockDim.x + threadIdx.x; e < total; e += gridDim.x * blockDim.x) {
    const unsigned xq = e % wq;
    unsigned t = e / wq;
    const int oy = (int)(t % (unsigned)Ho);
    t /= (unsigned)Ho;
    const int oz = (int)(t % (unsigned)Do);
    t /= (unsigned)Do;
    const int c = (int)(t % (unsigned)C);
    const int n = (int)(t / (unsigned)C);
    const LinTap tz = lin_tap(oz, rz, Di, align), ty = lin_tap(oy, ry, Hi, align);
    const float* p = x + ((long)n * C + c) * Di * Hi * Wi;
    const float* p00 = p + (long)tz.i0 * Hi * Wi + (long)ty.i0 * Wi;
    const float* p01 = p + (long)tz.i0 * Hi * Wi + (long)ty.i1 * Wi;
    const float* p10 = p + (long)tz.i1 * Hi * Wi + (long)ty.i0 * Wi;
    const float* p11 = p + (long)tz.i1 * Hi * Wi + (long)ty.i1 * Wi;
    float v[4];
#pragma unroll
    for (int k = 0; k < 4; ++k) {
      const LinTap tx = lin_tap((int)(xq * 4) + k, rx, Wi, align);
      v[k] = tz.l0 * (ty.l0 * (tx.l0 * p00[tx.i0] + tx.l1 * p00[tx.i1]) + ty.l1 * (tx.l0 * p01[tx.i0] + tx.l1 * p01[tx.i1])) +
             tz.l1 * (ty.l0 * (tx.l0 * p10[tx.i0] + tx.l1 * p10[tx.i1]) + ty.l1 * (tx.l0 * p11[tx.i0] + tx.l1 * p11[tx.i1]));
    }
    *reinterpret_cast<float4*>(y + (long)n * y_bstride + (((long)c * Do + oz) * Ho + oy) * Wo + xq * 4) = make_float4(v[0], v[1], v[2], v[3]);
  }
}

__device__ __forceinline__ float up2_even(float prev, float cur, bool first) { return first ? cur : 0.25f * prev + 0.75f * cur; }
__device__ __forceinline__ float up2_odd(float cur, float next) { return 0.75f * cur + 0.25f * next; }

__global__ __launch_bounds__(256) void upsample2x_fwd_kernel(const float* __restrict__ x, float* __restrict__ y, int N, int C, int Di,
                                                             int Hi, int Wi, long y_bstride, const float* __restrict__ ss) {
  const unsigned wq = (unsigned)Wi >> 1;
  const unsigned total = (unsigned)N * C * Di * Hi * wq;
  const int Ho = 2 * Hi, Wo = 2 * Wi;
  for (unsigned e = blockIdx.x * blockDim.x + threadIdx.x; e < total; e += gridDim.x * blockDim.x) {
    const unsigned xq = e % wq;
    unsigned t = e / wq;
    const int iy = (int)(t % (unsigned)Hi);
    t /= (unsigned)Hi;
    const int iz = (int)(t % (unsigned)Di);
    t /= (unsigned)Di;
    const int c = (int)(t % (unsigned)C);
    const int n = (int)(t / (unsigned)C);
    const float* p = x + ((long)n * C + c) * Di * Hi * Wi;
    const float sc = ss ? ss[2 * (n * C + c)] : 1.f, sh = ss ? ss[2 * (n * C + c) + 1] : 0.f;
    const int ix = (int)xq * 2;
    const int xa = ix > 0 ? ix - 1 : 0, xd = ix + 2 < Wi ? ix + 2 : Wi - 1;
    float r[3][3][4];
#pragma unroll
    for (int dz = 0; dz < 3; ++dz) {
      int z = iz + dz - 1;
      z = z < 0 ? 0 : (z > Di - 1 ? Di - 1 : z);
#pragma unroll
      for (int dy = 0; dy < 3; ++dy) {
        int yy = iy + dy - 1;
        yy = yy < 0 ? 0 : (yy > Hi - 1 ? Hi - 1 : yy);
        const float* row = p + ((long)z * Hi + yy) * Wi;
        float a = row[xa], b = row[ix], cc = row[ix + 1], d = row[xd];
        if (ss) { a = norm_relu1(a, sc, sh); b = norm_relu1(b, sc, sh); cc = norm_relu1(cc, sc, sh); d = norm_relu1(d, sc, sh); }
        r[dz][dy][0] = up2_even(a, b, ix == 0);
        r[dz][dy][1] = up2_odd(b, cc);
        r[dz][dy][2] = up2_even(b, cc, false);
        r[dz][dy][3] = up2_odd(cc, d);
      }
    }
    float u[3][2][4];
#pragma unroll
    for (int dz = 0; dz < 3; ++dz)
#pragma unroll
      for (int k = 0; k < 4; ++k) {
        u[dz][0][k] = up2_even(r[dz][0][k], r[dz][1][k], iy == 0);
        u[dz][1][k] = up2_odd(r[dz][1][k], r[dz][2][k]);
      }
    float* yo = y + (long)n * y_bstride + (((long)c * (2 * Di) + 2 * iz) * Ho + 2 * iy) * Wo + ix * 2;
#pragma unroll
    for (int py = 0; py < 2; ++py) {
      float ev[4], od[4];
#pragma unroll
      for (int k = 0; k < 4; ++k) {
        ev[k] = up2_even(u[0][py][k], u[1][py][k], iz == 0);
        od[k] = up2_odd(u[1][py][k], u[2][py][k]);
      }
      *reinterpret_cast<float4*>(yo + (long)py * Wo) = make_float4(ev[0], ev[1], ev[2], ev[3]);
      *reinterpret_cast<float4*>(yo + ((long)Ho + py) * Wo) = make_float4(od[0], od[1], od[2], od[3]);
    }
  }
}

__device__ __forceinline__ void up2_adj_weights(int i, int n, float w[4]) {
  w[0] = i > 0 ? 0.25f : 0.f;
  w[1] = i > 0 ? 0.75f : 1.f;
  w[2] = i < n - 1 ? 0.75f : 1.f;
  w[3] = i < n - 1 ? 0.25f : 0.f;
}

__global__ __launch_bounds__(256) void upsample2x_fwd_x4_kernel(const float* __restrict__ x, float* __restrict__ y, int N, int C, int Di,
                                                                int Hi, int Wi, long y_bstride, const float* __restrict__ ss) {
  const unsigned wq = (unsigned)Wi >> 2;
  const unsigned total = (unsigned)N * C * Di * Hi * wq;
  const int Ho = 2 * Hi, Wo = 2 * Wi;
  for (unsigned e = blockIdx.x * blockDim.x + threadIdx.x; e < total; e += gridDim.x * blockDim.x) {
    const unsigned xq = e % wq;
    unsigned t = e / wq;
    const int iy = (int)(t % (unsigned)Hi);
    t /= (unsigned)Hi;
    const int iz = (int)(t % (unsigned)Di);
    t /= (unsigned)Di;
    const int c = (int)(t % (unsigned)C);
// ... 327 lines not shown
```

### icl_amd/ops.py

```python
from __future__ import annotations

import ctypes
import math
import os
from typing import Optional, Sequence

import torch

from . import _lib
from .step_scope import BackwardEnd, DeferredBiasGrads, DeferredWgradReduce, FactoredGrads, ScopeField, StepScope, WgradLane

_vp = ctypes.c_void_p


def _ptr(t: Optional[torch.Tensor]):
    return None if t is None else _vp(t.data_ptr())


def _stream(t: torch.Tensor):
    if t.is_cuda:
        return _vp(torch.cuda.current_stream(t.device).cuda_stream)
    return None


# ... 369 lines not shown
        ctx.stats = conv3d_forward_raw(x, wp, bias, n, cin, cout, d, h, w, ks, cin * s, y, cout * s, wsplit=wsf, want_stats=want_stats)
        return y

    @staticmethod
    def backward(ctx, gy, gstats=None):
        if gy is None:
            return None, None, None, None, None
        x, weight = ctx.saved_tensors
        L = _lib.lib()
        gy = gy.contiguous()
        n, cin, d, h, w = x.shape
        cout, ks = weight.shape[0], weight.shape[2]
        s = d * h * w
        gx = gw = gb = None
        lane = (ks == 3 and WgradLane.wants(x, s) and ctx.needs_input_grad[0] and ctx.needs_input_grad[1] and not getattr(ctx, "cin1", False)
                and not (cin * 27 <= FIRST_CONV_PLANES_MAX_K))
        if lane:
            WgradLane.fork_point(gy)
        if ctx.needs_input_grad[0]:
            if ctx.pointwise_gemm:
                gx = torch.empty_like(x)
                gemm(weight, gy, cin, s, cout, cin, s, False, False, out=gx, ldc=s, batch=n, b_bstride=cout * s, c_bstride=cin * s)
            elif ctx.pointwise_small:
                gx = torch.empty_like(x)
                _lib.check(L.icl_conv1x1_small(_ptr(gy), _ptr(weight), None, _ptr(gx), n, cout, cin, s, 1, cin, _stream(x)),
                           "conv1x1_small dgrad")
            else:
                gx = torch.empty_like(x)
                wpt = ctx.wpt if ctx.wpt is not None else pack_weights(weight, 1)
                conv3d_forward_raw(gy, wpt, None, n, cout, cin, d, h, w, ks, cout * s, gx, cin * s, wsplit=getattr(ctx, "wsd", None))
        if ctx.needs_input_grad[1] or (ctx.has_bias and ctx.needs_input_grad[2]):
            gw = torch.empty_like(weight)
            gb = torch.empty(cout, dtype=torch.float32, device=x.device) if ctx.has_bias else None
            gb_arg = gb
            if ctx.has_bias and ctx.zero_bias_grad:
                gb = _cached_zeros(cout, x.device).view(cout) if getattr(StepScope.current, "packed", None) is not None else x.new_zeros(cout)
                gb_arg = None
            flops = 2.0 * ks ** 3 * cin * cout * s * n
            nbytes = 4.0 * (n * s * (cin + cout) + 2 * ks ** 3 * cin * cout)
            if ks == 1 and s % 4 == 0 and n * s >= CONV1X1_WGRAD_MIN_VOXELS:
                ws = _ws(L.icl_conv1x1_wgrad_ws_bytes(n, s, cin, cout), x)
                with _timed("conv1x1_wgrad_kernel", flops, nbytes, x):
                    _lib.check(L.icl_conv1x1_wgrad(_ptr(x), _ptr(gy), _ptr(gw), _ptr(gb_arg), _ptr(ws), n, cin, cout, s, cin * s,
                                                   cout * s, _stream(x)), "conv1x1_wgrad")
            elif getattr(ctx, "cin1", False) and w % 4 == 0 and gb_arg is None and gy.data_ptr() % 16 == 0:
                ws = _ws(L.icl_conv3d_cin1_wgrad_ws_bytes(n, d, h), x)
                with _timed("conv_cin1_wgrad_kernel", flops, nbytes, x):
                    _lib.check(L.icl_conv3d_cin1_wgrad(_ptr(x), _ptr(gy), _ptr(gw), _ptr(ws), n, cout, d, h, w, cin * s, cout * s,
                                                       _stream(x)), "conv3d_cin1_wgrad")
            elif ks == 3 and cin * 27 <= FIRST_CONV_PLANES_MAX_K and w % 4 == 0 and n * s >= CONV1X1_WGRAD_MIN_VOXELS * 64:
                planes = torch.empty((n, cin * 27, s), dtype=torch.float32, device=x.device)
                _lib.check(L.icl_im2col3_planes(_ptr(x), _ptr(planes), n, cin, d, h, w, _stream(x)), "im2col3_planes")
                ws = _ws(L.icl_conv1x1_wgrad_ws_bytes(n, s, cin * 27, cout), x)
                with _timed("conv1x1_wgrad_kernel", flops, nbytes, x):
                    _lib.check(L.icl_conv1x1_wgrad(_ptr(planes), _ptr(gy), _ptr(gw), _ptr(gb_arg), _ptr(ws), n, cin * 27, cout, s,
                                                   cin * 27 * s, cout * s, _stream(x)), "conv1x1_wgrad")
            else:
                tiny6 = ks == 3 and (d, h, w) == (6, 6, 6) and _f6_split_ok(x, weight)
                swap = (ks == 3 and gb_arg is None and cout == 16 and cin % 48 == 0 and h % 8 == 0 and d >= 8 and w % 4 == 0
                        and s >= WGRAD_SWAP_MIN_VOXELS and os.environ.get("ICL_WGRAD_SWAP", "1") != "0")

                def wgrad():
                    if tiny6:
                        cols = torch.empty((n * s, cin * 27), dtype=torch.float32, device=x.device)
                        _lib.check(L.icl_im2col3(_ptr(x), _ptr(cols), n, cin, d, h, w, _stream(x)), "im2col3")
                        g2 = gy.reshape(n, cout, s).transpose(1, 2).reshape(n * s, cout).contiguous()
                        gw2, gb2 = _tall_atb(g2, cols, gb_arg is not None)
                        gw.copy_(gw2.view_as(gw))
                        if gb_arg is not None:
                            gb_arg.copy_(gb2)
                        return
                    if swap:
                        ws = _ws(L.icl_conv3d_wgrad_ws_bytes(n, cout, cin, ks), x)
                        gws = torch.empty((cin, cout, ks, ks, ks), dtype=torch.float32, device=x.device)
                        with _timed("conv3d_mfma_wgrad_kernel", flops, nbytes, x):
                            _lib.check(L.icl_conv3d_wgrad(_ptr(gy), _ptr(x), _ptr(gws), None, _ptr(ws), n, cout, cin, d, h, w, ks,
                                                          cout * s, cin * s, _stream(x)), "conv3d_wgrad (roles exchanged)")
                        gw.copy_(gws.flip(2, 3, 4).transpose(0, 1))
                        return
                    ws = _ws(L.icl_conv3d_wgrad_ws_bytes(n, cin, cout, ks), x)
                    if gb_arg is None and DeferredWgradReduce.wants(weight):
                        ns = ctypes.c_int32(0)
                        with _timed("conv3d_mfma_wgrad_kernel", flops, nbytes, x):
                            _lib.check(L.icl_conv3d_wgrad_slabs(_ptr(x), _ptr(gy), _ptr(ws), n, cin, cout, d, h, w, ks, cin * s, cout * s,
                                                                ctypes.byref(ns), _stream(x)), "conv3d_wgrad_slabs")
                        DeferredWgradReduce.defer(ws, gw, cout, cin, ks, ns.value, weight)
                        return
                    with _timed("conv3d_mfma_wgrad_kernel", flops, nbytes, x):
                        _lib.check(L.icl_conv3d_wgrad(_ptr(x), _ptr(gy), _ptr(gw), _ptr(gb_arg), _ptr(ws), n, cin, cout, d, h, w, ks,
                                                      cin * s, cout * s, _stream(x)), "conv3d_wgrad")
                if lane:
                    with WgradLane.on_lane(x, gy, gw, gb_arg):
                        wgrad()
                    if not WgradLane.adoptable(weight):
                        WgradLane.sync_to_current(gw)
                else:
                    wgrad()
        return gx, gw, gb, None, None


class _Im2Col3(torch.autograd.Function):
    @staticmethod
    def forward(ctx, x):
        _require(x)
        L = _lib.lib()
        x = x.contiguous()
        n, c, d, h, w = x.shape
        cols = torch.empty((n * d * h * w, c * 27), dtype=torch.float32, device=x.device)
        _lib.check(L.icl_im2col3(_ptr(x), _ptr(cols), n, c, d, h, w, _stream(x)), "im2col3")
        ctx.shape = (n, c, d, h, w)
        return cols

    @staticmethod
    def backward(ctx, g):
        L = _lib.lib()
        n, c, d, h, w = ctx.shape
        g = g.contiguous()
        dx = torch.empty((n, c, d, h, w), dtype=torch.float32, device=g.device)
        _lib.check(L.icl_col2im3(_ptr(g), _ptr(dx), n, c, d, h, w, _stream(g)), "col2im3")
        return dx


SMALL_CONV_MAX_VOXELS = 216
WGRAD_SWAP_MIN_VOXELS = 24 ** 3
SMALL_CONV_MIN_WEIGHTS = 128 * 128 * 27


def _f6_split_ok(x, weight) -> bool:
    cout, cin = weight.shape[0], weight.shape[1]
    return (tuple(x.shape[2:]) == (6, 6, 6) and cin % 16 == 0 and cin >= 32 and ((cout + 15) // 16 * 16) % 32 == 0
            and os.environ.get("ICL_CONV_SPLIT", "1") != "0" and os.environ.get("ICL_CONV_SPLIT_FLAT6", "1") != "0"
            and os.environ.get("ICL_CONV_SPLIT_KSPLIT", "-1") != "0" and int(os.environ.get("ICL_CONV_SPLIT_MIN", 216)) <= 216)


def _conv3d_tiny_volume(x, weight, bias):
    n, cin, d, h, w = x.shape
    cout = weight.shape[0]
    y = linear(_Im2Col3.apply(x), weight.flatten(1), bias, lane_wgrad=True)
    return y.view(n, d * h * w, cout).permute(0, 2, 1).reshape(n, cout, d, h, w)


def conv3d(x: torch.Tensor, weight: torch.Tensor, bias: Optional[torch.Tensor] = None,
           zero_bias_grad: bool = False) -> torch.Tensor:
    if (weight.shape[2] == 3 and x.shape[2] * x.shape[3] * x.shape[4] <= SMALL_CONV_MAX_VOXELS
            and weight.numel() >= SMALL_CONV_MIN_WEIGHTS and not _f6_split_ok(x, weight)):
        return _conv3d_tiny_volume(x, weight, bias)
    return _Conv3d.apply(x, weight, bias, zero_bias_grad)


def conv3d_instance_norm_act(x: torch.Tensor, weight: torch.Tensor, bias: Optional[torch.Tensor], act: int = 1, eps: float = 1e-5):
    if (weight.shape[2] == 3 and x.shape[2] * x.shape[3] * x.shape[4] <= SMALL_CONV_MAX_VOXELS
            and weight.numel() >= SMALL_CONV_MIN_WEIGHTS and not _f6_split_ok(x, weight)):
        return _NormAct.apply(_conv3d_tiny_volume(x, weight, bias), None, None, None, None, 0, True, int(act), eps, 0.0, None)
    y, stats = _Conv3d.apply(x, weight, bias, True, True)
    return _NormAct.apply(y, None, None, None, None, 0, True, int(act), eps, 0.0, stats if stats.numel() else None)



class _NormAct(torch.autograd.Function):
    @staticmethod
    def forward(ctx, x, gamma, beta, running_mean, running_var, mode, use_batch_stats, act, eps, momentum, stats=None):
        _require(x, gamma, beta, running_mean, running_var)
        L = _lib.lib()
        x = x.contiguous()
        n, c = x.shape[0], x.shape[1]
        s = x.numel() // (n * c)
        groups = c if mode == 1 else n * c
        y = torch.empty_like(x)
        ws = _ws(L.icl_norm_ws_bytes(n, c, s), x)
        if use_batch_stats:
            mean = torch.empty(groups, dtype=torch.float32, device=x.device)
            rstd = torch.empty(groups, dtype=torch.float32, device=x.device)
            rm, rv = running_mean, running_var
        else:
            assert mode == 1 and running_mean is not None
            mean = running_mean.detach().clone()
            rstd = torch.empty(groups, dtype=torch.float32, device=x.device)
            _lib.check(L.icl_rstd_from_var(_ptr(running_var), _ptr(rstd), c, eps, _stream(x)), "rstd_from_var")
            rm = rv = None
        if stats is not None and use_batch_stats:
            assert mode == 0 and stats.shape[0] == n * c and stats.is_contiguous()
            _lib.check(L.icl_norm_fwd_given_stats(_ptr(x), None, _ptr(y), _ptr(mean), _ptr(rstd), _ptr(gamma), _ptr(beta), _ptr(rm), _ptr(rv),
                                                  n, c, s, mode, act, eps, momentum, _ptr(stats), stats.shape[1], _stream(x)),
                       "norm_fwd_given_stats")
        else:
            _lib.check(L.icl_norm_fwd(_ptr(x), _ptr(y), _ptr(mean), _ptr(rstd), _ptr(gamma), _ptr(beta), _ptr(rm), _ptr(rv),
                                      n, c, s, mode, int(use_batch_stats), act, eps, momentum, _ptr(ws), _stream(x)), "norm_fwd")
        ctx.save_for_backward(x, mean, rstd, gamma, beta)
        ctx.cfg = (mode, int(use_batch_stats), act)
        return y

    @staticmethod
    def backward(ctx, gy):
        x, mean, rstd, gamma, beta = ctx.saved_tensors
        mode, ubs, act = ctx.cfg
        L = _lib.lib()
        gy = gy.contiguous()
        n, c = x.shape[0], x.shape[1]
        s = x.numel() // (n * c)
        gx = torch.empty_like(x)
        dg = db = None
        if gamma is not None:
            dg = torch.empty_like(gamma)
            db = torch.empty_like(beta)
        ws = _ws(L.icl_norm_ws_bytes(n, c, s), x)
        _lib.check(L.icl_norm_bwd(_ptr(gy), _ptr(x), _ptr(mean), _ptr(rstd), _ptr(gamma), _ptr(beta), _ptr(gx), _ptr(dg),
                                  _ptr(db), n, c, s, mode, ubs, act, _ptr(ws), _stream(x)), "norm_bwd")
        return gx, dg, db, None, None, None, None, None, None, None, None


def instance_norm_relu(x: torch.Tensor, relu: bool = True, eps: float = 1e-5) -> torch.Tensor:
    return _NormAct.apply(x, None, None, None, None, 0, True, int(relu), eps, 0.0)


def instance_norm_act(x: torch.Tensor, act: int, eps: float = 1e-5) -> torch.Tensor:
    return _NormAct.apply(x, None, None, None, None, 0, True, int(act), eps, 0.0)



def _lazy_norm_min_voxels() -> int:
    if os.environ.get("ICL_LAZY_NORM", "1") == "0":
        return 1 << 62
    return int(os.environ.get("ICL_LAZY_NORM_MIN", str(48 ** 3)))


class LazyAct:
    __slots__ = ("t", "ss")

    def __init__(self, t: torch.Tensor, ss: torch.Tensor):
        self.t, self.ss = t, ss

    @property
    def shape(self):
        return self.t.shape

    def materialize(self) -> torch.Tensor:
        return _LazyMaterialize.apply(self.t, self.ss)


def materialized(x):
    return x.materialize() if isinstance(x, LazyAct) else x


class _NormActLazy(torch.autograd.Function):

    @staticmethod
    def forward(ctx, y, stats, eps):
        _require(y, stats)
        L = _lib.lib()
        n, c = y.shape[0], y.shape[1]
        mean = torch.empty(n * c, dtype=torch.float32, device=y.device)
        rstd = torch.empty(n * c, dtype=torch.float32, device=y.device)
        ss = torch.empty((n * c, 2), dtype=torch.float32, device=y.device)
        _lib.check(L.icl_norm_finalize_stats(_ptr(stats), n, c, stats.shape[1], eps, _ptr(mean), _ptr(rstd), _ptr(ss), _stream(y)),
                   "norm_finalize_stats")
        ctx.save_for_backward(y, mean, rstd)
        ctx.mark_non_differentiable(ss)
        ctx.set_materialize_grads(False)
        return y.view_as(y), ss

    @staticmethod
    def backward(ctx, ga, gss=None):
        if ga is None:
            return None, None, None
        y, mean, rstd = ctx.saved_tensors
        L = _lib.lib()
        ga = ga.contiguous()
        n, c = y.shape[0], y.shape[1]
        s = y.numel() // (n * c)
        gy = torch.empty_like(y)
        ws = _ws(L.icl_norm_ws_bytes(n, c, s), y)
        _lib.check(L.icl_norm_bwd(_ptr(ga), _ptr(y), _ptr(mean), _ptr(rstd), None, None, _ptr(gy), None, None, n, c, s, 0, 1, 1, _ptr(ws),
                                  _stream(y)), "norm_bwd")
        return gy, None, None


class _LazyMaterialize(torch.autograd.Function):
    @staticmethod
    def forward(ctx, t, ss):
        L = _lib.lib()
        n, c = t.shape[0], t.shape[1]
        s = t.numel() // (n * c)
        if s % 4:
            sc = ss[:, 0].reshape(n, c, *([1] * (t.dim() - 2)))
            sh = ss[:, 1].reshape(n, c, *([1] * (t.dim() - 2)))
            return torch.clamp_min(torch.addcmul(sh, t, sc), 0.0)
        out = torch.empty_like(t)
        _lib.check(L.icl_norm_apply(_ptr(t), _ptr(ss), _ptr(out), n, c, s, _stream(t)), "norm_apply")
        return out

    @staticmethod
    def backward(ctx, g):
        return g, None


def conv3d_instance_norm_act_lazy(x: torch.Tensor, weight: torch.Tensor, bias: Optional[torch.Tensor], eps: float = 1e-5):
    s = x.shape[2] * x.shape[3] * x.shape[4]
    if weight.shape[2] != 3 or s < _lazy_norm_min_voxels() or s % 4 or not torch.is_grad_enabled():
        return conv3d_instance_norm_act(x, weight, bias, act=1, eps=eps)
    y, stats = _Conv3d.apply(x, weight, bias, True, True)
    if not stats.numel():
        return _NormAct.apply(y, None, None, None, None, 0, True, 1, eps, 0.0, None)
    av, ss = _NormActLazy.apply(y, stats, eps)
    return LazyAct(av, ss)


class _InstanceNormAddAct(torch.autograd.Function):

    @staticmethod
    def forward(ctx, x, res, act, eps, stats=None):
        _require(x, res)
        L = _lib.lib()
        x, res = x.contiguous(), res.contiguous()
        assert x.shape == res.shape
        n, c = x.shape[0], x.shape[1]
        s = x.numel() // (n * c)
        y = torch.empty_like(x)
        mean = torch.empty(n * c, dtype=torch.float32, device=x.device)
        rstd = torch.empty(n * c, dtype=torch.float32, device=x.device)
        if stats is not None:
            assert stats.shape[0] == n * c and stats.is_contiguous()
            _lib.check(L.icl_norm_fwd_given_stats(_ptr(x), _ptr(res), _ptr(y), _ptr(mean), _ptr(rstd), None, None, None, None, n, c, s, 0, act,
                                                  eps, 0.0, _ptr(stats), stats.shape[1], _stream(x)), "norm_fwd_given_stats")
        else:
            ws = _ws(L.icl_norm_ws_bytes(n, c, s), x)
            _lib.check(L.icl_norm_res_fwd(_ptr(x), _ptr(res), _ptr(y), _ptr(mean), _ptr(rstd), None, None, None, None, n, c, s, 0, 1, act,
                                          eps, 0.0, _ptr(ws), _stream(x)), "norm_res_fwd")
        ctx.save_for_backward(x, res, mean, rstd)
        ctx.act = act
        return y

    @staticmethod
    def backward(ctx, gy):
        x, res, mean, rstd = ctx.saved_tensors
        L = _lib.lib()
        gy = gy.contiguous()
        n, c = x.shape[0], x.shape[1]
        s = x.numel() // (n * c)
        gx = torch.empty_like(x)
        gres = torch.empty_like(x)
        ws = _ws(L.icl_norm_ws_bytes(n, c, s), x)
        _lib.check(L.icl_norm_res_bwd(_ptr(gy), _ptr(x), _ptr(res), _ptr(mean), _ptr(rstd), None, None, _ptr(gx), _ptr(gres), None,
                                      None, n, c, s, 0, 1, ctx.act, _ptr(ws), _stream(x)), "norm_res_bwd")
        return gx, gres, None, None, None


def instance_norm_add_act(x: torch.Tensor, res: torch.Tensor, act: int = 2, eps: float = 1e-5) -> torch.Tensor:
    return _InstanceNormAddAct.apply(x, res, int(act), eps)


def conv3d_instance_norm_add_act(x: torch.Tensor, weight: torch.Tensor, res: torch.Tensor, act: int = 2, eps: float = 1e-5) -> torch.Tensor:
    if (weight.shape[2] == 3 and x.shape[2] * x.shape[3] * x.shape[4] <= SMALL_CONV_MAX_VOXELS
            and weight.numel() >= SMALL_CONV_MIN_WEIGHTS and not _f6_split_ok(x, weight)):
        return _InstanceNormAddAct.apply(_conv3d_tiny_volume(x, weight, None), res, int(act), eps)
    y, stats = _Conv3d.apply(x, weight, None, True, True)
    return _InstanceNormAddAct.apply(y, res, int(act), eps, stats if stats.numel() else None)


def batch_norm_relu(x, gamma, beta, running_mean, running_var, training: bool, relu: bool = True,
                    eps: float = 1e-5, momentum: float = 0.1) -> torch.Tensor:
    return _NormAct.apply(x, gamma, beta, running_mean, running_var, 1, bool(training), int(relu), eps, momentum)


def batch_norm_act(x, gamma, beta, running_mean, running_var, training: bool, act: int,
                   eps: float = 1e-5, momentum: float = 0.1) -> torch.Tensor:
    return _NormAct.apply(x, gamma, beta, running_mean, running_var, 1, bool(training), int(act), eps, momentum)


def _embed_2d_weight(weight: torch.Tensor) -> torch.Tensor:
    co, ci, kh, kw = weight.shape
    if kh == 1:
        return weight.unsqueeze(2)
    w3 = weight.new_zeros((co, ci, 3, kh, kw))
    w3[:, :, 1] = weight
    return w3


def conv2d(x: torch.Tensor, weight: torch.Tensor, bias: Optional[torch.Tensor] = None, zero_bias_grad: bool = False) -> torch.Tensor:
    return conv3d(x.unsqueeze(2), _embed_2d_weight(weight), bias, zero_bias_grad).squeeze(2)


def depthwise_conv2d(x: torch.Tensor, weight: torch.Tensor) -> torch.Tensor:
    return depthwise_conv3d(x.unsqueeze(2), _embed_2d_weight(weight)).squeeze(2)



class _MaxPool2(torch.autograd.Function):
    @staticmethod
    def forward(ctx, x, pd):
        _require(x)
        L = _lib.lib()
        x = x.contiguous()
        n, c, d, h, w = x.shape
        assert d % pd == 0 and h % 2 == 0 and w % 2 == 0, "max-pool kernels need even extents"
        y = torch.empty((n, c, d // pd, h // 2, w // 2), dtype=torch.float32, device=x.device)
        idx = torch.empty(y.shape, dtype=torch.uint8, device=x.device)
        _lib.check(L.icl_maxpool2_fwd(_ptr(x), _ptr(y), _ptr(idx), n * c, d // pd, h // 2, w // 2, pd, _stream(x)), "maxpool2_fwd")
        ctx.save_for_backward(idx)
        ctx.pd = pd
        return y

    @staticmethod
    def backward(ctx, gy):
        (idx,) = ctx.saved_tensors
        L = _lib.lib()
        gy = gy.contiguous()
        n, c, d, h, w = gy.shape
        gx = torch.empty((n, c, d * ctx.pd, h * 2, w * 2), dtype=torch.float32, device=gy.device)
        _lib.check(L.icl_maxpool2_bwd(_ptr(gy), _ptr(idx), _ptr(gx), n * c, d, h, w, ctx.pd, _stream(gy)), "maxpool2_bwd")
        return gx, None


class _SkipAndPool(torch.autograd.Function):

    @staticmethod
    def forward(ctx, x):
        _require(x)
        L = _lib.lib()
        x = x.contiguous()
        n, c, d, h, w = x.shape
        assert d % 2 == 0 and h % 2 == 0 and w % 2 == 0, "max-pool kernels need even extents"
        y = torch.empty((n, c, d // 2, h // 2, w // 2), dtype=torch.float32, device=x.device)
        idx = torch.empty(y.shape, dtype=torch.uint8, device=x.device)
        _lib.check(L.icl_maxpool2_fwd(_ptr(x), _ptr(y), _ptr(idx), n * c, d // 2, h // 2, w // 2, 2, _stream(x)), "maxpool2_fwd")
        ctx.save_for_backward(idx)
        return x.view_as(x), y

    @staticmethod
    def backward(ctx, gskip, gy):
        (idx,) = ctx.saved_tensors
        L = _lib.lib()
        n, c, d, h, w = idx.shape
        if gy is None:
            return gskip
        gy = gy.contiguous()
        gx = torch.empty((n, c, d * 2, h * 2, w * 2), dtype=torch.float32, device=gy.device)
        plane = 8 * d * h * w
        ok = (gskip is not None and gskip.dtype == torch.float32 and tuple(gskip.shape) == tuple(gx.shape)
              and gskip.stride()[1:] == (plane, 4 * h * w, 2 * w, 1) and gskip.stride(0) % 2 == 0 and gskip.data_ptr() % 8 == 0)
        if ok:
            _lib.check(L.icl_maxpool2_bwd_add(_ptr(gy), _ptr(idx), _vp(gskip.data_ptr()), _ptr(gx), n, c, d, h, w, 2, gskip.stride(0),
                                              _stream(gy)), "maxpool2_bwd_add")
            return gx
        _lib.check(L.icl_maxpool2_bwd(_ptr(gy), _ptr(idx), _ptr(gx), n * c, d, h, w, 2, _stream(gy)), "maxpool2_bwd")
        return gx if gskip is None else gx + gskip


class _SkipAndPoolLazy(torch.autograd.Function):

    @staticmethod
    def forward(ctx, t, ss):
        L = _lib.lib()
        n, c, d, h, w = t.shape
        y = torch.empty((n, c, d // 2, h // 2, w // 2), dtype=torch.float32, device=t.device)
        idx = torch.empty(y.shape, dtype=torch.uint8, device=t.device)
        _lib.check(L.icl_maxpool2_fwd_norm(_ptr(t), _ptr(ss), _ptr(y), _ptr(idx), n * c, d // 2, h // 2, w // 2, 2, _stream(t)), "maxpool2_fwd_norm")
        ctx.save_for_backward(idx)
        return t.view_as(t), y

    @staticmethod
    def backward(ctx, gskip, gy):
        return _SkipAndPool.backward(ctx, gskip, gy), None


def skip_and_pool(x):
    if isinstance(x, LazyAct):
        d, h, w = x.t.shape[2:]
        if d % 2 == 0 and h % 2 == 0 and w % 2 == 0 and x.t.is_contiguous():
            skip, pooled = _SkipAndPoolLazy.apply(x.t, x.ss)
            return LazyAct(skip, x.ss), pooled
        x = x.materialize()
    return _SkipAndPool.apply(x)


def max_pool3d_2(x: torch.Tensor) -> torch.Tensor:
    return _MaxPool2.apply(x, 2)


def max_pool2d_2(x: torch.Tensor) -> torch.Tensor:
    return _MaxPool2.apply(x.unsqueeze(2), 1).squeeze(2)



class _Trilinear(torch.autograd.Function):
    @staticmethod
    def forward(ctx, x, size, align):
        _require(x)
        L = _lib.lib()
        x = x.contiguous()
        n, c, di, hi, wi = x.shape
        do, ho, wo = size
        y = torch.empty((n, c, do, ho, wo), dtype=torch.float32, device=x.device)
        _lib.check(L.icl_trilinear_fwd(_ptr(x), _ptr(y), n, c, di, hi, wi, do, ho, wo, c * do * ho * wo, align, _stream(x)),
                   "trilinear_fwd")
        ctx.in_shape = (n, c, di, hi, wi)
        ctx.align = align
        return y

    @staticmethod
    def backward(ctx, gy):
        L = _lib.lib()
        gy = gy.contiguous()
        n, c, di, hi, wi = ctx.in_shape
        do, ho, wo = gy.shape[2:]
        gx = torch.empty(ctx.in_shape, dtype=torch.float32, device=gy.device)
        ws = _ws(L.icl_trilinear_bwd_ws_bytes(n, c, di, hi, wi, do, ho, wo), gy)
        _lib.check(L.icl_trilinear_bwd(_ptr(gy), _ptr(gx), _ptr(ws), n, c, di, hi, wi, do, ho, wo, c * do * ho * wo, ctx.align,
                                       _stream(gy)), "trilinear_bwd")
        return gx, None, None


def trilinear_resize(x: torch.Tensor, size: Sequence[int], align_corners: bool = False) -> torch.Tensor:
    return _Trilinear.apply(x, tuple(int(s) for s in size), int(bool(align_corners)))


def bilinear_resize(x: torch.Tensor, size: Sequence[int], align_corners: bool = False) -> torch.Tensor:
    return _Trilinear.apply(x.unsqueeze(2), (1, int(size[0]), int(size[1])), int(bool(align_corners))).squeeze(2)


class _UpCat(torch.autograd.Function):

    @staticmethod
    def forward(ctx, skip, deep):
        _require(skip, deep)
        L = _lib.lib()
        skip = skip.contiguous()
        deep = deep.contiguous()
        n, cs, d, h, w = skip.shape
        cd = deep.shape[1]
        assert deep.shape[0] == n and tuple(deep.shape[2:]) == (d // 2, h // 2, w // 2)
        s = d * h * w
        out = torch.empty((n, cs + cd, d, h, w), dtype=torch.float32, device=skip.device)
        _lib.check(L.icl_copy_rows(_ptr(skip), _ptr(out), n, cs * s, cs * s, (cs + cd) * s, _stream(skip)), "copy_rows")
        up_view = out[:, cs:]
        _lib.check(L.icl_trilinear_fwd(_ptr(deep), _vp(up_view.data_ptr()), n, cd, d // 2, h // 2, w // 2, d, h, w,
                                       (cs + cd) * s, 0, _stream(skip)), "trilinear_fwd")
        ctx.dims = (n, cs, cd, d, h, w)
        return out

    @staticmethod
    def backward(ctx, g):
        L = _lib.lib()
        g = g.contiguous()
        n, cs, cd, d, h, w = ctx.dims
        s = d * h * w
        gskip = gdeep = None
        if ctx.needs_input_grad[0]:
            gskip = g[:, :cs]
        if ctx.needs_input_grad[1]:
            gdeep = torch.empty((n, cd, d // 2, h // 2, w // 2), dtype=torch.float32, device=g.device)
            gv = g[:, cs:]
            ws = _ws(L.icl_trilinear_bwd_ws_bytes(n, cd, d // 2, h // 2, w // 2, d, h, w), g)
            _lib.check(L.icl_trilinear_bwd(_vp(gv.data_ptr()), _ptr(gdeep), _ptr(ws), n, cd, d // 2, h // 2, w // 2, d, h, w,
                                           (cs + cd) * s, 0, _stream(g)), "trilinear_bwd")
        return gskip, gdeep


class _UpCatLazy(torch.autograd.Function):

    @staticmethod
    def forward(ctx, skip, skip_ss, deep, deep_ss):
        L = _lib.lib()
        n, cs, d, h, w = skip.shape
        cd = deep.shape[1]
        out = torch.empty((n, cs + cd, d, h, w), dtype=torch.float32, device=skip.device)
        _lib.check(L.icl_upsample2x_concat_norm(_ptr(skip), _ptr(skip_ss), _ptr(deep), _ptr(deep_ss), _ptr(out), n, cs, cd, d, h, w,
                                                _stream(skip)), "upsample2x_concat_norm")
        ctx.dims = (n, cs, cd, d, h, w)
        return out

    @staticmethod
    def backward(ctx, g):
        ctx2 = ctx
        needs = ctx.needs_input_grad

        class _View:
            dims = ctx2.dims
            needs_input_grad = (needs[0], needs[2])
        gskip, gdeep = _UpCat.backward(_View, g)
        return gskip, None, gdeep, None


def upsample2x_concat(skip, deep) -> torch.Tensor:
    if isinstance(skip, LazyAct) or isinstance(deep, LazyAct):
        st, dt = (skip.t if isinstance(skip, LazyAct) else skip), (deep.t if isinstance(deep, LazyAct) else deep)
        n, cs, d, h, w = st.shape
        ok = (d % 2 == 0 and h % 2 == 0 and w % 4 == 0 and tuple(dt.shape[2:]) == (d // 2, h // 2, w // 2) and dt.shape[0] == n
              and st.is_contiguous() and dt.is_contiguous() and st.dtype == torch.float32 and (st.is_cuda or _lib.host_pointers_ok()))
        if ok:
            return _UpCatLazy.apply(st, skip.ss if isinstance(skip, LazyAct) else None, dt, deep.ss if isinstance(deep, LazyAct) else None)
        skip, deep = materialized(skip), materialized(deep)
    return _UpCat.apply(skip, deep)



class _DWConv3(torch.autograd.Function):
    @staticmethod
    def forward(ctx, x, weight):
        _require(x, weight)
        L = _lib.lib()
        x = x.contiguous()
        weight = weight.contiguous()
        n, c, d, h, w = x.shape
        assert tuple(weight.shape) == (c, 1, 3, 3, 3)
        y = torch.empty_like(x)
        _lib.check(L.icl_dwconv3_fwd(_ptr(x), _ptr(weight), _ptr(y), n, c, d, h, w, 0, _stream(x)), "dwconv3_fwd")
        ctx.save_for_backward(x, weight)
        return y

    @staticmethod
    def backward(ctx, gy):
        x, weight = ctx.saved_tensors
        L = _lib.lib()
        gy = gy.contiguous()
        n, c, d, h, w = x.shape
        gx = gw = None
        if ctx.needs_input_grad[0]:
            gx = torch.empty_like(x)
            _lib.check(L.icl_dwconv3_fwd(_ptr(gy), _ptr(weight), _ptr(gx), n, c, d, h, w, 1, _stream(x)), "dwconv3_dgrad")
        if ctx.needs_input_grad[1]:
            gw = torch.empty_like(weight)
            ws = _ws(L.icl_dwconv3_wgrad_ws_bytes(n, c, d, h, w), x)
# ... 1203 lines not shown
```

### include/icl_hip.h

```cpp
#ifndef ICL_HIP_H
#define ICL_HIP_H
#include <stdint.h>
#ifdef __cplusplus
extern "C" {
#endif

int icl_abi_version(void);
const char* icl_last_error(void);
const char* icl_last_kernel_name(void);

int64_t icl_conv3d_packed_elems(int cout, int cin, int ks, int mode);
int icl_conv3d_pack_weights(const float* w, float* wp, int cout, int cin, int ks, int mode, void* stream);
int icl_conv3d_pack_weights_both(const float* w, float* wp_fwd, float* wp_dgrad, int cout, int cin, int ks, void* stream);
int icl_conv3d_pack_weights_multi(const void* const* w, void* const* wp_fwd, void* const* wp_dgrad, const int32_t* cout, const int32_t* cin,
                                  const int32_t* ks, int count, void* stream);
int64_t icl_conv3d_fwd_ws_bytes(int n, int cin, int cout, int d, int h, int w, int ks);
int64_t icl_conv3d_split_ws_bytes(int cin, int cout);
int icl_conv3d_split_weights_multi(const void* const* wp, void* const* wsplit, const int32_t* cin, const int32_t* cout, int count,
                                   void* stream);
int icl_conv3d_fwd_presplit(const float* x, const void* wsplit, const float* bias, float* y, int n, int cin, int cout, int d, int h, int w,
                            int64_t x_bstride, int64_t y_bstride, void* stream);
int64_t icl_conv3d_fwd_presplit_ws_bytes(int n, int cin, int cout, int d, int h, int w);
int icl_conv3d_fwd_presplit_ws(const float* x, const void* wsplit, const float* bias, float* y, void* ws, int n, int cin, int cout, int d,
                               int h, int w, int64_t x_bstride, int64_t y_bstride, void* stream);
int icl_conv3d_fwd_stats_slots(int n, int cin, int cout, int d, int h, int w);
int icl_conv3d_fwd_presplit_stats(const float* x, const void* wsplit, const float* bias, float* y, float* stats, int n, int cin, int cout,
                                  int d, int h, int w, int64_t x_bstride, int64_t y_bstride, void* stream);
int icl_conv3d_fwd(const float* x, const float* wp, const float* bias, float* y, void* ws, int n, int cin, int cout, int d, int h,
                   int w, int ks, int64_t x_bstride, int64_t y_bstride, void* stream);
int64_t icl_conv3d_wgrad_ws_bytes(int n, int cin, int cout, int ks);
int icl_conv3d_wgrad(const float* x, const float* gy, float* gw, float* gbias, void* ws, int n, int cin, int cout, int d,
                     int h, int w, int ks, int64_t x_bstride, int64_t gy_bstride, void* stream);
int icl_conv3d_wgrad_slabs(const float* x, const float* gy, void* ws, int n, int cin, int cout, int d, int h, int w, int ks,
                           int64_t x_bstride, int64_t gy_bstride, int32_t* nslabs, void* stream);
int icl_conv3d_wgrad_reduce_multi(const void* const* ws, void* const* gw, const int32_t* cout, const int32_t* cin, const int32_t* ks,
                                  const int32_t* nslabs, int count, void* stream);

int64_t icl_norm_ws_bytes(int n, int c, int64_t s);
int icl_norm_fwd(const float* x, float* y, float* mean, float* rstd, const float* gamma, const float* beta,
                 float* running_mean, float* running_var, int n, int c, int64_t s, int mode, int use_batch_stats,
                 int act, float eps, float momentum, void* ws, void* stream);
int icl_norm_bwd(const float* gy, const float* x, const float* mean, const float* rstd, const float* gamma,
                 const float* beta, float* gx, float* dgamma, float* dbeta, int n, int c, int64_t s, int mode,
                 int use_batch_stats, int act, void* ws, void* stream);
int icl_norm_fwd_given_stats(const float* x, const float* res, float* y, float* mean, float* rstd, const float* gamma, const float* beta,
                             float* running_mean, float* running_var, int n, int c, int64_t s, int mode, int act, float eps,
                             float momentum, const float* part, int nslots, void* stream);
int icl_norm_res_fwd(const float* x, const float* res, float* y, float* mean, float* rstd, const float* gamma, const float* beta,
                     float* running_mean, float* running_var, int n, int c, int64_t s, int mode, int use_batch_stats,
                     int act, float eps, float momentum, void* ws, void* stream);
int icl_norm_res_bwd(const float* gy, const float* x, const float* res, const float* mean, const float* rstd, const float* gamma,
                     const float* beta, float* gx, float* gres, float* dgamma, float* dbeta, int n, int c, int64_t s, int mode,
                     int use_batch_stats, int act, void* ws, void* stream);
int icl_rstd_from_var(const float* var, float* rstd, int c, float eps, void* stream);

int icl_norm_finalize_stats(const float* part, int n, int c, int nslots, float eps, float* mean, float* rstd, float* ss, void* stream);
int icl_norm_apply(const float* x, const float* ss, float* y, int n, int c, int64_t s, void* stream);
int icl_maxpool2_fwd_norm(const float* x, const float* ss, float* y, uint8_t* idx, int64_t nc, int dout, int hout, int wout, int pool_depth,
                          void* stream);
int icl_upsample2x_concat_norm(const float* skip, const float* skip_ss, const float* deep, const float* deep_ss, float* out, int n, int cs,
                               int cd, int d, int h, int w, void* stream);

int icl_maxpool2_fwd(const float* x, float* y, uint8_t* idx, int64_t nc, int dout, int hout, int wout, int pool_depth, void* stream);
int icl_maxpool2_bwd(const float* gy, const uint8_t* idx, float* gx, int64_t nc, int dout, int hout, int wout, int pool_depth, void* stream);
int icl_maxpool2_bwd_add(const float* gy, const uint8_t* idx, const float* add, float* gx, int n, int c, int dout, int hout, int wout,
                         int pool_depth, int64_t add_bstride, void* stream);

int icl_trilinear_fwd(const float* x, float* y, int n, int c, int di, int hi, int wi, int dout, int hout, int wout,
                      int64_t y_bstride, int align_corners, void* stream);
int64_t icl_trilinear_bwd_ws_bytes(int n, int c, int di, int hi, int wi, int dout, int hout, int wout);
int icl_trilinear_bwd(const float* gy, float* gx, void* ws, int n, int c, int di, int hi, int wi, int dout, int hout, int wout,
                      int64_t gy_bstride, int align_corners, void* stream);

int icl_copy_rows(const float* src, float* dst, int64_t rows, int64_t row_elems, int64_t src_stride, int64_t dst_stride,
                  void* stream);

int icl_concat2(const float* a, int64_t na, const float* b, int64_t nb, float* out, void* stream);

int icl_dwconv3_fwd(const float* x, const float* w, float* y, int n, int c, int d, int h, int wd, int flip, void* stream);
int64_t icl_dwconv3_wgrad_ws_bytes(int n, int c, int d, int h, int wd);
int icl_dwconv3_wgrad(const float* x, const float* gy, float* gw, void* ws, int n, int c, int d, int h, int wd, void* stream);

int icl_conv1x1_small(const float* x, const float* w, const float* bias, float* y, int n, int cin, int cout, int64_t s, int w_ostride,
                      int w_istride, void* stream);
int icl_conv1x1_dropout(const float* x, const float* w, const float* bias, float* y, int n, int cin, int cout, int64_t s, int w_ostride,
                        int w_istride, int mask_mode, uint32_t seed, float p, const uint32_t* seed_dev, void* stream);
int icl_conv1x1_wgrad_dropout(const float* x, const float* gy, float* gw, float* gbias, void* ws, int n, int cin, int cout, int64_t s,
                              int64_t gy_bstride, uint32_t seed, float p, const uint32_t* seed_dev, void* stream);
int icl_conv1x1_dropout_norm(const float* x, const float* ss, const float* w, const float* bias, float* y, int n, int cin, int cout, int64_t s,
                             int w_ostride, int w_istride, uint32_t seed, float p, const uint32_t* seed_dev, void* stream);
int icl_conv1x1_wgrad_dropout_norm(const float* x, const float* ss, const float* gy, float* gw, float* gbias, void* ws, int n, int cin,
                                   int cout, int64_t s, int64_t gy_bstride, uint32_t seed, float p, const uint32_t* seed_dev, void* stream);

int icl_dropout(const float* x, float* y, int64_t n, uint32_t seed, float p, const uint32_t* seed_dev, void* stream);
int icl_drop_path(const float* x, float* y, int64_t n, int64_t group, uint32_t seed, float p, const uint32_t* seed_dev, void* stream);
int icl_drop_path_add(const float* x, const float* res, float* y, int64_t n, int64_t group, uint32_t seed, float p,
                      const uint32_t* seed_dev, void* stream);

#define ICL_LOSS_MAX_BLOCKS 1024
#define ICL_LOSS_STATS_FLOATS(nc) ((3 * (nc) + 1) * (1 + ICL_LOSS_MAX_BLOCKS))
int icl_loss_fwd(const float* a, const float* b, const int64_t* labels, const float* weight, float* stats, float* out,
                 int batch, int nc, int64_t s, int mode, int a_is_prob, void* stream);
int icl_loss_bwd(const float* a, const float* b, const int64_t* labels, const float* weight, const float* stats,
                 const float* gout0, const float* gout1, float* ga, int batch, int nc, int64_t s, int mode, int a_is_prob,
                 void* stream);
typedef struct IclLossJob {
  const float* a; const float* b; const int64_t* labels; const float* weight;
  float* stats; float* out;
  const float* gout0; const float* gout1; float* ga;
  int64_t s;
  int batch, nc, mode, a_is_prob;
} IclLossJob;
int icl_loss_fwd_multi(const IclLossJob* jobs, int count, void* stream);
int icl_loss_bwd_multi(const IclLossJob* jobs, int count, void* stream);

int icl_layernorm_fwd(const float* x, const float* gamma, const float* beta, float* y, float* mean, float* rstd, int64_t rows,
                      int c, float eps, void* stream);
int64_t icl_layernorm_bwd_ws_bytes(int64_t rows, int c);
int icl_layernorm_bwd(const float* gy, const float* x, const float* gamma, const float* mean, const float* rstd, float* gx,
                      float* dgamma, float* dbeta, void* ws, int64_t rows, int c, void* stream);
int icl_gelu_fwd(const float* x, float* y, int64_t n, void* stream);
int icl_gelu_bwd(const float* gy, const float* x, float* gx, int64_t n, void* stream);
int icl_attn_fwd(const float* q, const float* kv, float* logits, float* out, float* stats, int b, int h, int nc, int n, int d,
                 float scale, void* stream);
int icl_attn_bwd(const float* q, const float* kv, const float* logits, const float* stats, const float* out, const float* gout,
                 const float* glog, float* gq, float* gkv, int b, int h, int nc, int n, int d, float scale, void* stream);
int64_t icl_attn_bwd_ws_bytes(int b, int h, int nc, int n, int d);
int icl_attn_bwd_ws(const float* q, const float* kv, const float* logits, const float* stats, const float* out, const float* gout,
                    const float* glog, float* gq, float* gkv, void* ws, int b, int h, int nc, int n, int d, float scale, void* stream);

int icl_colsum_multi(const void* const* g, void* const* out, const int32_t* rows, const int32_t* cols, int count, void* stream);
int icl_scalar_combine(const void* const* in, const float* w, int n_in, int n_out, float* out, void* stream);

int icl_gather_rows(const float* src, const int32_t* idx, float* out, int64_t b, int64_t s, int64_t m, int c, void* stream);
int icl_gather_rows_sum2(const float* src, const int32_t* idx2, float* out, int64_t b, int64_t s, int64_t m, int c, void* stream);

int icl_im2col3(const float* x, float* cols, int n, int c, int d, int h, int w, void* stream);
int icl_im2col3_planes(const float* x, float* planes, int n, int c, int d, int h, int w, void* stream);

int icl_conv3d_cin1_fwd(const float* x, const float* w, const float* bias, float* y, int n, int cout, int d, int h, int wd, int64_t x_bstride,
                        int64_t y_bstride, void* stream);
int64_t icl_conv3d_cin1_wgrad_ws_bytes(int n, int d, int h);
int icl_conv3d_cin1_wgrad(const float* x, const float* gy, float* gw, void* ws, int n, int cout, int d, int h, int wd, int64_t x_bstride,
                          int64_t gy_bstride, void* stream);
int icl_col2im3(const float* g, float* dx, int n, int c, int d, int h, int w, void* stream);

int icl_depth_to_space2(const float* yt, float* out, int n, int d, int h, int w, int cout, int64_t out_bstride, void* stream);
int icl_space_to_depth2(const float* g, float* gt, int n, int d, int h, int w, int cout, int64_t g_bstride, void* stream);

int64_t icl_linear_ws_bytes(int64_t rows, int in, int out, int kind);
int icl_linear_fwd(const float* x, const float* w, const float* bias, float* y, void* ws, int64_t rows, int in, int out, int act,
                   void* stream);
int icl_linear_dgrad(const float* gy, const float* w, float* gx, void* ws, int64_t rows, int in, int out, void* stream);
int icl_linear_bwd_small(const float* gy, const float* w, const float* x, float* gx, float* dw, void* ws, int64_t rows, int in, int out,
                         void* stream);
int icl_linear_wgrad_small(const float* gy, const float* x, float* dw, void* ws, int64_t rows, int in, int out, void* stream);
int icl_linear_dgrad_sgd(const float* gy, const float* x, float* w, float* mom, float* gx, void* ws, int64_t rows, int in, int out,
                         float lr, float momentum, float weight_decay, int first, const float* lr_dev, void* stream);
int64_t icl_gemm_ws_bytes(int64_t m, int n, int k, int batch);
int icl_gemm(const float* a, const float* b, float* c, const float* bias, void* ws, int64_t m, int n, int k, int64_t lda, int64_t ldb,
             int64_t ldc, int a_kcontig, int b_kcontig, int act, int batch, int64_t a_bstride, int64_t b_bstride, int64_t c_bstride,
             void* stream);

int64_t icl_linear_wgrad_ws_bytes(int64_t rows, int o, int i);
int icl_linear_wgrad(const float* gy, const float* x, float* dw, float* db, void* ws, int64_t rows, int o, int i, void* stream);

int64_t icl_conv1x1_wgrad_ws_bytes(int n, int64_t s, int cin, int cout);
int icl_conv1x1_wgrad(const float* x, const float* gy, float* gw, float* gbias, void* ws, int n, int cin, int cout, int64_t s,
                      int64_t x_bstride, int64_t gy_bstride, void* stream);

int64_t icl_window_attn_bias_elems(int n, int heads);
int icl_relpos_bias_fwd(const float* table, const int64_t* index, float* bias, int n, int heads, int idx_stride, void* stream);
int icl_window_attn_fwd(const float* qkv, const float* bias, const int32_t* regions, float* out, float* lse, int b_, int n, int heads,
                        int nw, int head_dim, float scale, void* stream);
int icl_window_attn_bwd(const float* qkv, const float* bias, const int32_t* regions, const float* out, const float* lse,
                        const float* dout, float* dqkv, float* dbias, int b_, int n, int heads, int nw, int head_dim, float scale,
                        void* stream);
int icl_window_attn_bwd_chunks(int b_, int n, int heads, int nw, int head_dim);
int icl_relpos_bias_bwd_sum(float* dbias, int chunks, const int32_t* inv, const int32_t* offs, float* dtable, int64_t table_rows, int n,
                            int heads, void* stream);

int icl_crop_rotflip(const void* const* images, const void* const* labels, const int32_t* params, int batch, float* image_out,
                     int64_t* label_out, int o0, int o1, int o2, void* stream);

int icl_sgd_step(float* p, const float* g, float* m, int64_t n, float lr, float momentum, float weight_decay, int first,
                 const float* lr_dev, void* stream);
int icl_sgd_step_factored(float* p, float* m, const float* g, const float* x, int rows, int n, int k, float lr, float momentum,
                          float weight_decay, int first, const float* lr_dev, void* stream);
int64_t icl_sgd_factored_split_ws_bytes(int rows, int n, int k);
int icl_sgd_step_factored_split(float* p, float* m, const float* g, const float* x, void* ws, int rows, int n, int k, float lr,
                                float momentum, float weight_decay, int first, const float* lr_dev, void* stream);
int icl_sgd_step_factored_narrow(float* p, float* m, const float* g, const float* x, int rows, int n, int k, float lr, float momentum,
                                 float weight_decay, int first, const float* lr_dev, int workgroups, void* stream);
int icl_sgd_step_multi(void* const* p, const void* const* g, void* const* m, const int64_t* n, int count, float lr,
                       float momentum, float weight_decay, int first, const float* lr_dev, void* stream);

typedef struct IclQcStage {
  const float* x; int x_rows;
  const float* w; const float* bias; float* y;
  int R, K, N, trans, nc, npw;
  int pro, epi;
  const float* pa; const float* pb; const float* pc; const float* pd; int pro_dp;
  float* so0; float* so1; float* so2;
  const float* ea; const float* eb; int ea_r0, ea_r1, eb_r0, eb_r1;
  uint32_t dp_seed[2], dp_thresh[2]; float dp_scale[2]; const uint32_t* dp_seed_dev;
  float eps;
} IclQcStage;
int icl_qchain_stage(const IclQcStage* stage, void* stream);
int icl_qchain_wgrad(const void* const* g, const void* const* x, void* const* dw, void* const* db, const int32_t* rows, const int32_t* n,
                     const int32_t* k, const int32_t* kind, int count, void* stream);

int64_t icl_seg_metrics_ws_bytes(int n0, int n1, int n2, int num_classes);
int icl_seg_metrics(const void* pred, int pred_dtype, const void* gt, int gt_dtype, int n0, int n1, int n2, int num_classes, int all_border,
                    int64_t* out, void* ws, void* stream);

#ifdef __cplusplus
}
#endif
#endif
```

Baseline: 203.2 volumes/s.

## Fuse norm-backward reductions into maxpool backward and cin1 conv wgrad

Adds a maxpool2 backward-add kernel that also computes the per-channel instance-norm backward partial sums (sum of masked grad and grad·xhat). The following lazy norm backward then consumes these sums and skips its own reduction pass. It also adds a fused first-layer (Cin=1) conv+norm+ReLU path whose weight-gradient kernel applies the norm/ReLU backward inline, so no separate gradient tensor is materialized. This saves full-volume reads and writes at the cost of extra plumbing, saved tensors and handoff state checked through tensor version tracking.

```diff
diff --git a/icl_amd/_lib.py b/icl_amd/_lib.py
--- a/icl_amd/_lib.py
+++ b/icl_amd/_lib.py
@@ -41,6 +41,9 @@
     "icl_norm_ws_bytes": (c_int64, [I, I, L]),
     "icl_norm_fwd": (c_int, [P, P, P, P, P, P, P, P, I, I, L, I, I, I, F, F, P, P]),
     "icl_norm_bwd": (c_int, [P, P, P, P, P, P, P, P, P, I, I, L, I, I, I, P, P]),
+    "icl_norm_bwd_given_sums": (c_int, [P, P, P, P, P, I, P, I, I, L, I, P]),
+    "icl_maxpool2_bwd_add_sums_slots": (c_int, [I, I, I]),
+    "icl_maxpool2_bwd_add_sums": (c_int, [P, P, P, P, P, P, P, P, I, I, I, I, I, L, P]),
     "icl_norm_res_fwd": (c_int, [P, P, P, P, P, P, P, P, P, I, I, L, I, I, I, F, F, P, P]),
     "icl_norm_res_bwd": (c_int, [P, P, P, P, P, P, P, P, P, P, P, I, I, L, I, I, I, P, P]),
     "icl_rstd_from_var": (c_int, [P, P, I, F, P]),
@@ -79,6 +82,8 @@
     "icl_conv3d_cin1_fwd": (c_int, [P, P, P, P, I, I, I, I, I, L, L, P]),
     "icl_conv3d_cin1_wgrad_ws_bytes": (c_int64, [I, I, I]),
     "icl_conv3d_cin1_wgrad": (c_int, [P, P, P, P, I, I, I, I, I, L, L, P]),
+    "icl_conv3d_cin1_norm_wgrad_ws_bytes": (c_int64, [I, I, I, I, I]),
+    "icl_conv3d_cin1_norm_wgrad": (c_int, [P, P, P, P, P, P, I, P, P, I, I, I, I, I, L, P]),
     "icl_col2im3": (c_int, [P, P, I, I, I, I, I, P]),
     "icl_linear_ws_bytes": (c_int64, [L, I, I, I]),
     "icl_linear_fwd": (c_int, [P, P, P, P, P, L, I, I, I, P]),
diff --git a/icl_amd/csrc/icl_abi.inc b/icl_amd/csrc/icl_abi.inc
--- a/icl_amd/csrc/icl_abi.inc
+++ b/icl_amd/csrc/icl_abi.inc
@@ -1168,6 +1168,17 @@
   return check_launch("norm_bwd_apply");
 }
 
+int icl_norm_bwd_given_sums(const float* gy, const float* x, const float* mean, const float* rstd, const float* part, int nslots, float* gx,
+                            int n, int c, int64_t s, int act, void* stream) {
+  if (!gy || !x || !mean || !rstd || !part || !gx || nslots < 1 || n < 1 || c < 1 || s < 1) return fail(-1, "norm_bwd_given_sums: bad argument");
+  const int R = n * c;
+  const int nch = (int)((s + icl::kNormChunk - 1) / icl::kNormChunk);
+  ICL_LAUNCH(icl::norm_act_bwd_apply_kernel, dim3(nch, R), dim3(icl::kNormThreads), 0, (hipStream_t)stream, gy, x, mean, rstd, (const float*)nullptr,
+             (const float*)nullptr, part, gx, (long)s, c, 0, act, 1.0f / (float)s, 1, (const float*)nullptr, (float*)nullptr, R, nslots,
+             (float*)nullptr, (float*)nullptr);
+  return check_launch("norm_bwd_apply (given sums)");
+}
+
 int icl_rstd_from_var(const float* var, float* rstd, int c, float eps, void* stream) {
   if (!var || !rstd || c < 1) return fail(-1, "rstd_from_var: bad argument");
   ICL_LAUNCH(icl::rstd_from_var_kernel, dim3((c + 63) / 64), dim3(64), 0, (hipStream_t)stream, var, rstd, c, eps);
@@ -1260,6 +1271,26 @@
   ICL_LAUNCH(icl::maxpool2_bwd_add_kernel, dim3(grid_for(total, 256)), dim3(256), 0, (hipStream_t)stream, gy, idx, add, gx, (long)n * c, c, dout,
              hout, wout, pool_depth, (long)add_bstride);
   return check_launch("maxpool2_bwd_add");
+}
+
+int icl_maxpool2_bwd_add_sums_slots(int dout, int hout, int wout) {
+  if (dout < 1 || hout < 1 || wout < 2 || (wout & 1)) return 0;
+  const long pairs = (long)dout * hout * (wout >> 1);
+  if (pairs % 256) return 0;
+  const long wgs = pairs / 256;
+  return (int)((wgs & 1) ? wgs : wgs / 2);
+}
+
+int icl_maxpool2_bwd_add_sums(const float* gy, const uint8_t* idx, const float* add, float* gx, const float* xraw, const float* mean,
+                              const float* rstd, float* part, int n, int c, int dout, int hout, int wout, int64_t add_bstride, void* stream) {
+  const int nslots = icl_maxpool2_bwd_add_sums_slots(dout, hout, wout);
+  if (!gy || !gx || !idx || !add || !xraw || !mean || !rstd || !part || n < 1 || c < 1 || nslots < 1 || (long)n * c > 65535 || (add_bstride & 3) ||
+      !aligned16(add) || !aligned16(gx) || !aligned16(xraw) || ((uintptr_t)gy & 7))
+    return fail(-1, "maxpool2_bwd_add_sums: bad argument (see icl_maxpool2_bwd_add_sums_slots; 16-byte aligned add / gx / xraw)");
+  const long wgs = (long)dout * hout * (wout >> 1) / 256;
+  ICL_LAUNCH(icl::maxpool2_bwd_add_x2_sums_kernel, dim3(nslots, n * c), dim3(256), 0, (hipStream_t)stream, gy, idx, add, gx, xraw, mean, rstd, part, c,
+             dout, hout, wout, (long)add_bstride, (int)(wgs / nslots), nslots);
+  return check_launch("maxpool2_bwd_add_x2_sums");
 }
 
 namespace {
@@ -1844,6 +1875,40 @@
   return check_launch("conv3d_cin1_wgrad_reduce");
 }
 
+int64_t icl_conv3d_cin1_norm_wgrad_ws_bytes(int n, int cout, int d, int h, int w) {
+  const int64_t s = (int64_t)d * h * w, nch = (s + icl::kNormChunk - 1) / icl::kNormChunk;
+  return icl_conv3d_cin1_wgrad_ws_bytes(n, d, h) + ((int64_t)n * cout * nch * 2 + (int64_t)n * cout * 4 + 64) * 4;
+}
+
+int icl_conv3d_cin1_norm_wgrad(const float* x, const float* gz, const float* y, const float* mean, const float* rstd, const float* sums,
+                               int nslots, float* gw, void* ws, int n, int cout, int d, int h, int wd, int64_t x_bstride, void* stream) {
+  icl::Cin1Geom g;
+  const long s = (long)d * h * wd;
+  if (!x || !gz || !y || !mean || !rstd || !gw || !ws || (sums && nslots < 1) || (wd & 3) || !aligned16(gz) || !aligned16(y) ||
+      !cin1_geom(g, n, cout, d, h, wd, x_bstride, (int64_t)cout * s))
+    return fail(-1, "conv3d_cin1_norm_wgrad: bad argument (W a multiple of 4, dense 16-byte aligned gz / y)");
+  hipStream_t st = (hipStream_t)stream;
+  const int R = n * cout;
+  const int grid = cin1_grid(g);
+  float* cpart = (float*)ws;
+  float* npart = cpart + (size_t)grid * 512;
+  if (!sums) {
+    nslots = (int)((s + icl::kNormChunk - 1) / icl::kNormChunk);
+    ICL_LAUNCH(icl::norm_act_bwd_partial_kernel, dim3(nslots, R), dim3(icl::kNormThreads), 0, st, gz, y, mean, rstd, (const float*)nullptr,
+               (const float*)nullptr, npart, s, cout, nslots, 0, 1, (const float*)nullptr);
+    if (int rc = check_launch("norm_bwd_partial")) return rc;
+    sums = npart;
+  }
+  float* quad = npart + (((size_t)R * ((s + icl::kNormChunk - 1) / icl::kNormChunk) * 2 + 3) & ~(size_t)3);
+  ICL_LAUNCH(icl::norm_bwd_merge_sums_kernel, dim3(R), dim3(64), 0, st, sums, nslots, mean, rstd, 1.0f / (float)s, quad);
+  if (int rc = check_launch("norm_bwd_merge_sums")) return rc;
+  ICL_LAUNCH(icl::conv_cin1_norm_wgrad_kernel, dim3(grid), dim3(icl::kC1Threads), cin1_lds(g), st, x, gz, y, (const float*)quad, cpart, g);
+  if (int rc = check_launch("conv3d_cin1_norm_wgrad")) return rc;
+  ICL_LAUNCH(icl::conv_cin1_wgrad_reduce_kernel, dim3(16), dim3(256), 0, st, (const float*)cpart, gw, grid, cout);
+  snprintf(g_kernel, sizeof(g_kernel), "conv_cin1_norm_wgrad_kernel");
+  return check_launch("conv3d_cin1_wgrad_reduce");
+}
+
 int64_t icl_conv1x1_wgrad_ws_bytes(int n, int64_t s, int cin, int cout) { return icl_linear_wgrad_ws_bytes((int64_t)n * s, cout, cin); }
 
 namespace {
diff --git a/icl_amd/csrc/kernels/conv_cin1.h b/icl_amd/csrc/kernels/conv_cin1.h
--- a/icl_amd/csrc/kernels/conv_cin1.h
+++ b/icl_amd/csrc/kernels/conv_cin1.h
@@ -23,8 +23,9 @@
   }
 }
 
-__global__ __launch_bounds__(kC1Threads) void conv_cin1_wgrad_kernel(const float* __restrict__ x, const float* __restrict__ gy,
-                                                                     float* __restrict__ part, Cin1Geom g) {
+template <bool NORM>
+__device__ __forceinline__ void c1_wgrad_body(const float* __restrict__ x, const float* __restrict__ gy, float* __restrict__ part, const Cin1Geom& g,
+                                              const float* __restrict__ yraw, const float* __restrict__ nrm) {
   ICL_DYN_LDS(float, xs);
   const int lane = threadIdx.x & 63, wid = threadIdx.x >> 6, lr = lane & 15, lg = lane >> 4;
   const int PW = g.W + 2, PR = kC1Rows + 2;
@@ -45,6 +46,9 @@
     c1_stage_halo(xs, x, g, n, z, y0);
     __syncthreads();
     const float* gb = gy + (long)n * g.y_bstride + (long)lr * DHW + (long)z * HW;
+    const float* yb = NORM ? yraw + (long)n * g.y_bstride + (long)lr * DHW + (long)z * HW : nullptr;
+    float4 nv = make_float4(0.f, 0.f, 0.f, 0.f);
+    if (NORM && lr < g.Cout) nv = *reinterpret_cast<const float4*>(nrm + ((long)n * g.Cout + lr) * 4);
     for (int rr = 0; rr < 2; ++rr) {
       const int ty = 2 * wid + rr, yy = y0 + ty;
       if (yy >= g.H) break;
@@ -53,8 +57,19 @@
       for (int x0 = 0; x0 < g.W; x0 += 16) {
         const int xl = x0 + 4 * lg;
         float4 a = make_float4(0.f, 0.f, 0.f, 0.f);
-        if (lr < g.Cout && xl < g.W) a = *reinterpret_cast<const float4*>(grow + xl);
-        const float av[4] = {a.x, a.y, a.z, a.w};
+        const bool ld = lr < g.Cout && xl < g.W;
+        if (ld) a = *reinterpret_cast<const float4*>(grow + xl);
+        float av[4] = {a.x, a.y, a.z, a.w};
+        if (NORM && ld) {
+          const float4 yv = *reinterpret_cast<const float4*>(yb + (long)yy * g.W + xl);
+          const float ys[4] = {yv.x, yv.y, yv.z, yv.w};
+#pragma unroll
+          for (int j = 0; j < 4; ++j) {
+            const float xh = (ys[j] - nv.x) * nv.y;
+            const float h = (xh > 0.f) ? av[j] : 0.f;
+            av[j] = nv.y * (h - nv.z - xh * nv.w);
+          }
+        }
         const bool in = xl < g.W;
 #pragma unroll
         for (int j = 0; j < 4; ++j) {
@@ -85,6 +100,17 @@
         part[(long)blockIdx.x * 512 + (4 * lg + r) * 32 + 16 * tb + lr] = s;
       }
   }
+}
+
+__global__ __launch_bounds__(kC1Threads) void conv_cin1_wgrad_kernel(const float* __restrict__ x, const float* __restrict__ gy,
+                                                                     float* __restrict__ part, Cin1Geom g) {
+  c1_wgrad_body<false>(x, gy, part, g, nullptr, nullptr);
+}
+
+__global__ __launch_bounds__(kC1Threads) void conv_cin1_norm_wgrad_kernel(const float* __restrict__ x, const float* __restrict__ gy,
+                                                                          const float* __restrict__ yraw, const float* __restrict__ nrm,
+                                                                          float* __restrict__ part, Cin1Geom g) {
+  c1_wgrad_body<true>(x, gy, part, g, yraw, nrm);
 }
 
 __global__ __launch_bounds__(256) void conv_cin1_wgrad_reduce_kernel(const float* __restrict__ part, float* __restrict__ gw, int nparts, int cout) {
diff --git a/icl_amd/csrc/kernels/norm.h b/icl_amd/csrc/kernels/norm.h
--- a/icl_amd/csrc/kernels/norm.h
+++ b/icl_amd/csrc/kernels/norm.h
@@ -226,6 +226,23 @@
   if (threadIdx.x == 0) {
     float* p = part + (r * nchunks + blockIdx.x) * 2;
     p[0] = p1; p[1] = p2;
+  }
+}
+
+__global__ __launch_bounds__(64) void norm_bwd_merge_sums_kernel(const float* __restrict__ part, int nchunks, const float* __restrict__ mean,
+                                                                 const float* __restrict__ rstd, float inv_count, float* __restrict__ out) {
+  const long r = blockIdx.x;
+  float p1 = 0.f, p2 = 0.f;
+  for (int it = threadIdx.x; it < nchunks; it += 64) {
+    const float* p = part + (r * nchunks + it) * 2;
+    p1 += p[0];
+    p2 += p[1];
+  }
+  p1 = wave_sum(p1);
+  p2 = wave_sum(p2);
+  if (threadIdx.x == 0) {
+    float* o = out + r * 4;
+    o[0] = mean[r]; o[1] = rstd[r]; o[2] = p1 * inv_count; o[3] = p2 * inv_count;
   }
 }
 
diff --git a/icl_amd/csrc/kernels/pool_resize.h b/icl_amd/csrc/kernels/pool_resize.h
--- a/icl_amd/csrc/kernels/pool_resize.h
+++ b/icl_amd/csrc/kernels/pool_resize.h
@@ -144,6 +144,59 @@
   }
 }
 
+__global__ __launch_bounds__(256) void maxpool2_bwd_add_x2_sums_kernel(const float* __restrict__ gy, const unsigned char* __restrict__ idx,
+                                                                       const float* __restrict__ add, float* __restrict__ gx,
+                                                                       const float* __restrict__ xraw, const float* __restrict__ mean,
+                                                                       const float* __restrict__ rstd, float* __restrict__ part, int C, int Do,
+                                                                       int Ho, int Wo, long add_bstride, int iters, int nslots) {
+  const int Wo2 = Wo >> 1;
+  const int H = Ho * 2, W = Wo * 2;
+  const long nc = blockIdx.y;
+  const long pairs = (long)Do * Ho * Wo2;
+  const long plane = (long)Do * 2 * H * W;
+  const float m = mean[nc], rs = rstd[nc];
+  const float* ab = add + (nc / C) * add_bstride + (nc % C) * plane;
+  const float* xb = xraw + nc * plane;
+  float* pb = gx + nc * plane;
+  float p1 = 0.f, p2 = 0.f;
+  for (int it = 0; it < iters; ++it) {
+    const long o2 = ((long)blockIdx.x * iters + it) * 256 + threadIdx.x;
+    if (o2 >= pairs) break;
+    const int ox = (int)(o2 % Wo2) * 2;
+    long t = o2 / Wo2;
+    const int oy = (int)(t % Ho);
+    const int oz = (int)(t / Ho);
+    const long o = nc * (pairs * 2) + ((long)oz * Ho + oy) * (long)Wo + ox;
+    const long in_plane = ((long)(oz * 2) * H + oy * 2) * (long)W + ox * 2;
+    const float2 g = *reinterpret_cast<const float2*>(gy + o);
+    const int b0 = idx[o], b1 = idx[o + 1];
+#pragma unroll
+    for (int k = 0; k < 8; k += 2) {
+      const long off = in_plane + ((k >> 2) * H + ((k >> 1) & 1)) * (long)W;
+      const float4 s = *reinterpret_cast<const float4*>(ab + off);
+      const float4 xv = *reinterpret_cast<const float4*>(xb + off);
+      const float4 v = make_float4(s.x + (b0 == k ? g.x : 0.f), s.y + (b0 == k + 1 ? g.x : 0.f),
+                                   s.z + (b1 == k ? g.y : 0.f), s.w + (b1 == k + 1 ? g.y : 0.f));
+      *reinterpret_cast<float4*>(pb + off) = v;
+      const float xs[4] = {xv.x, xv.y, xv.z, xv.w}, vs[4] = {v.x, v.y, v.z, v.w};
+#pragma unroll
+      for (int q = 0; q < 4; ++q) {
+        const float xh = (xs[q] - m) * rs;
+        const float h = (xh > 0.f) ? vs[q] : 0.f;
+        p1 += h;
+        p2 += h * xh;
+      }
+    }
+  }
+  __shared__ float red[256 / 64];
+  p1 = block_sum<256>(p1, red);
+  p2 = block_sum<256>(p2, red);
+  if (threadIdx.x == 0) {
+    float* p = part + (nc * nslots + blockIdx.x) * 2;
+    p[0] = p1; p[1] = p2;
+  }
+}
+
 struct LinTap { int i0, i1; float l0, l1; };
 __device__ __forceinline__ LinTap lin_tap(int dst, float rscale, int in_size, int align) {
   float src = align ? rscale * (float)dst : rscale * ((float)dst + 0.5f) - 0.5f;
diff --git a/icl_amd/ops.py b/icl_amd/ops.py
--- a/icl_amd/ops.py
+++ b/icl_amd/ops.py
@@ -545,8 +545,86 @@
     if (weight.shape[2] == 3 and x.shape[2] * x.shape[3] * x.shape[4] <= SMALL_CONV_MAX_VOXELS
             and weight.numel() >= SMALL_CONV_MIN_WEIGHTS and not _f6_split_ok(x, weight)):
         return _NormAct.apply(_conv3d_tiny_volume(x, weight, bias), None, None, None, None, 0, True, int(act), eps, 0.0, None)
+    if _Conv3dCin1NormAct.wants(x, weight, act):
+        return _Conv3dCin1NormAct.apply(x, weight, bias, eps)
     y, stats = _Conv3d.apply(x, weight, bias, True, True)
     return _NormAct.apply(y, None, None, None, None, 0, True, int(act), eps, 0.0, stats if stats.numel() else None)
+
+
+def _norm_bwd_sums_on() -> bool:
+    return os.environ.get("ICL_NORM_BWD_SUMS", "1") != "0"
+
+
+class NormBwdSums:
+    __slots__ = ("mean", "rstd", "_gx", "_version", "_part")
+    launches = 0
+
+    def __init__(self):
+        self.mean = self.rstd = self._gx = self._part = None
+        self._version = -1
+
+    def offer(self, gx: torch.Tensor, part: torch.Tensor):
+        self._gx, self._version, self._part = gx, gx._version, part
+
+    def take(self, ga: torch.Tensor):
+        gx, version, part = self._gx, self._version, self._part
+        self._gx = self._part = None
+        if gx is None or ga is not gx or ga._version != version:
+            return None
+        NormBwdSums.launches += 1
+        return part
+
+
+class _Conv3dCin1NormAct(torch.autograd.Function):
+
+    @staticmethod
+    def wants(x, weight, act) -> bool:
+        return (int(act) == 1 and weight.shape[2] == 3 and weight.shape[1] == 1 and weight.shape[0] <= 16 and x.dim() == 5
+                and x.shape[4] % 4 == 0 and 120 * (x.shape[4] + 2) <= 65536 and not x.requires_grad and weight.requires_grad
+                and torch.is_grad_enabled() and os.environ.get("ICL_CONV_CIN1", "1") != "0" and _norm_bwd_sums_on())
+
+    @staticmethod
+    def forward(ctx, x, weight, bias, eps):
+        _require(x, weight, bias)
+        L = _lib.lib()
+        x, weight = x.contiguous(), weight.contiguous()
+        n, _, d, h, w = x.shape
+        cout = weight.shape[0]
+        s = d * h * w
+        WgradLane.note_use(weight)
+        y = torch.empty((n, cout, d, h, w), dtype=torch.float32, device=x.device)
+        with _timed("conv_cin1_fwd_kernel", 2.0 * 27 * cout * s * n, 4.0 * n * s * (1 + cout), x):
+            _lib.check(L.icl_conv3d_cin1_fwd(_ptr(x), _ptr(weight), _ptr(bias), _ptr(y), n, cout, d, h, w, s, cout * s, _stream(x)),
+                       "conv3d_cin1_fwd")
+        z = torch.empty_like(y)
+        mean = torch.empty(n * cout, dtype=torch.float32, device=x.device)
+        rstd = torch.empty(n * cout, dtype=torch.float32, device=x.device)
+        ws = _ws(L.icl_norm_ws_bytes(n, cout, s), x)
+        _lib.check(L.icl_norm_fwd(_ptr(y), _ptr(z), _ptr(mean), _ptr(rstd), None, None, None, None, n, cout, s, 0, 1, 1, eps, 0.0, _ptr(ws),
+                                  _stream(x)), "norm_fwd")
+        ctx.save_for_backward(x, weight, y, mean, rstd)
+        ctx.has_bias = bias is not None
+        return z
+
+    @staticmethod
+    def backward(ctx, gz):
+        x, weight, y, mean, rstd = ctx.saved_tensors
+        L = _lib.lib()
+        gz = gz.contiguous()
+        if gz.data_ptr() % 16:
+            gz = gz.clone()
+        n, _, d, h, w = x.shape
+        cout = weight.shape[0]
+        s = d * h * w
+        gw = torch.empty_like(weight)
+        ws = _ws(L.icl_conv3d_cin1_norm_wgrad_ws_bytes(n, cout, d, h, w), x)
+        with _timed("conv_cin1_norm_wgrad_kernel", 2.0 * 27 * cout * s * n, 4.0 * n * s * (1 + 4 * cout), x):
+            _lib.check(L.icl_conv3d_cin1_norm_wgrad(_ptr(x), _ptr(gz), _ptr(y), _ptr(mean), _ptr(rstd), None, 0, _ptr(gw), _ptr(ws), n, cout,
+                                                    d, h, w, s, _stream(x)), "conv3d_cin1_norm_wgrad")
+        gb = None
+        if ctx.has_bias:
+            gb = _cached_zeros(cout, x.device).view(cout) if getattr(StepScope.current, "packed", None) is not None else x.new_zeros(cout)
+        return None, gw, gb, None
 
 
 
@@ -618,10 +696,10 @@
 
 
 class LazyAct:
-    __slots__ = ("t", "ss")
-
-    def __init__(self, t: torch.Tensor, ss: torch.Tensor):
-        self.t, self.ss = t, ss
+    __slots__ = ("t", "ss", "req")
+
+    def __init__(self, t: torch.Tensor, ss: torch.Tensor, req: Optional["NormBwdSums"] = None):
+        self.t, self.ss, self.req = t, ss, req
 
     @property
     def shape(self):
@@ -638,7 +716,7 @@
 class _NormActLazy(torch.autograd.Function):
 
     @staticmethod
-    def forward(ctx, y, stats, eps):
+    def forward(ctx, y, stats, eps, req=None):
         _require(y, stats)
         L = _lib.lib()
         n, c = y.shape[0], y.shape[1]
@@ -650,22 +728,30 @@
         ctx.save_for_backward(y, mean, rstd)
         ctx.mark_non_differentiable(ss)
         ctx.set_materialize_grads(False)
+        ctx.req = req
+        if req is not None:
+            req.mean, req.rstd = mean, rstd
         return y.view_as(y), ss
 
     @staticmethod
     def backward(ctx, ga, gss=None):
         if ga is None:
-            return None, None, None
+            return None, None, None, None
         y, mean, rstd = ctx.saved_tensors
         L = _lib.lib()
-        ga = ga.contiguous()
         n, c = y.shape[0], y.shape[1]
         s = y.numel() // (n * c)
         gy = torch.empty_like(y)
+        part = ctx.req.take(ga) if ctx.req is not None else None
+        if part is not None:
+            _lib.check(L.icl_norm_bwd_given_sums(_ptr(ga), _ptr(y), _ptr(mean), _ptr(rstd), _ptr(part), part.shape[1], _ptr(gy), n, c, s, 1,
+                                                 _stream(y)), "norm_bwd_given_sums")
+            return gy, None, None, None
+        ga = ga.contiguous()
         ws = _ws(L.icl_norm_ws_bytes(n, c, s), y)
         _lib.check(L.icl_norm_bwd(_ptr(ga), _ptr(y), _ptr(mean), _ptr(rstd), None, None, _ptr(gy), None, None, n, c, s, 0, 1, 1, _ptr(ws),
                                   _stream(y)), "norm_bwd")
-        return gy, None, None
+        return gy, None, None, None
 
 
 class _LazyMaterialize(torch.autograd.Function):
@@ -694,8 +780,9 @@
     y, stats = _Conv3d.apply(x, weight, bias, True, True)
     if not stats.numel():
         return _NormAct.apply(y, None, None, None, None, 0, True, 1, eps, 0.0, None)
-    av, ss = _NormActLazy.apply(y, stats, eps)
-    return LazyAct(av, ss)
+    req = NormBwdSums() if _norm_bwd_sums_on() else None
+    av, ss = _NormActLazy.apply(y, stats, eps, req)
+    return LazyAct(av, ss, req)
 
 
 class _InstanceNormAddAct(torch.autograd.Function):
@@ -821,7 +908,7 @@
 
     @staticmethod
     def backward(ctx, gskip, gy):
-        (idx,) = ctx.saved_tensors
+        idx = ctx.saved_tensors[0]
         L = _lib.lib()
         n, c, d, h, w = idx.shape
         if gy is None:
@@ -831,6 +918,18 @@
         plane = 8 * d * h * w
         ok = (gskip is not None and gskip.dtype == torch.float32 and tuple(gskip.shape) == tuple(gx.shape)
               and gskip.stride()[1:] == (plane, 4 * h * w, 2 * w, 1) and gskip.stride(0) % 2 == 0 and gskip.data_ptr() % 8 == 0)
+        req = getattr(ctx, "req", None)
+        if (ok and req is not None and req.mean is not None and len(ctx.saved_tensors) == 2 and StepScope.current is not None
+                and _norm_bwd_sums_on() and gskip.stride(0) % 4 == 0 and gskip.data_ptr() % 16 == 0 and n * c <= 65535):
+            slots = L.icl_maxpool2_bwd_add_sums_slots(d, h, w)
+            if slots:
+                t = ctx.saved_tensors[1]
+                part = torch.empty((n * c, slots, 2), dtype=torch.float32, device=gy.device)
+                _lib.check(L.icl_maxpool2_bwd_add_sums(_ptr(gy), _ptr(idx), _vp(gskip.data_ptr()), _ptr(gx), _ptr(t), _ptr(req.mean),
+                                                       _ptr(req.rstd), _ptr(part), n, c, d, h, w, gskip.stride(0), _stream(gy)),
+                           "maxpool2_bwd_add_sums")
+                req.offer(gx, part)
+                return gx
         if ok:
             _lib.check(L.icl_maxpool2_bwd_add(_ptr(gy), _ptr(idx), _vp(gskip.data_ptr()), _ptr(gx), n, c, d, h, w, 2, gskip.stride(0),
                                               _stream(gy)), "maxpool2_bwd_add")
@@ -842,25 +941,29 @@
 class _SkipAndPoolLazy(torch.autograd.Function):
 
     @staticmethod
-    def forward(ctx, t, ss):
+    def forward(ctx, t, ss, req=None):
         L = _lib.lib()
         n, c, d, h, w = t.shape
         y = torch.empty((n, c, d // 2, h // 2, w // 2), dtype=torch.float32, device=t.device)
         idx = torch.empty(y.shape, dtype=torch.uint8, device=t.device)
         _lib.check(L.icl_maxpool2_fwd_norm(_ptr(t), _ptr(ss), _ptr(y), _ptr(idx), n * c, d // 2, h // 2, w // 2, 2, _stream(t)), "maxpool2_fwd_norm")
-        ctx.save_for_backward(idx)
+        ctx.req = req
+        if req is not None:
+            ctx.save_for_backward(idx, t)
+        else:
+            ctx.save_for_backward(idx)
         return t.view_as(t), y
 
     @staticmethod
     def backward(ctx, gskip, gy):
-        return _SkipAndPool.backward(ctx, gskip, gy), None
+        return _SkipAndPool.backward(ctx, gskip, gy), None, None
 
 
 def skip_and_pool(x):
     if isinstance(x, LazyAct):
         d, h, w = x.t.shape[2:]
         if d % 2 == 0 and h % 2 == 0 and w % 2 == 0 and x.t.is_contiguous():
-            skip, pooled = _SkipAndPoolLazy.apply(x.t, x.ss)
+            skip, pooled = _SkipAndPoolLazy.apply(x.t, x.ss, x.req)
             return LazyAct(skip, x.ss), pooled
         x = x.materialize()
     return _SkipAndPool.apply(x)
diff --git a/include/icl_hip.h b/include/icl_hip.h
--- a/include/icl_hip.h
+++ b/include/icl_hip.h
@@ -53,6 +53,8 @@
                      const float* beta, float* gx, float* gres, float* dgamma, float* dbeta, int n, int c, int64_t s, int mode,
                      int use_batch_stats, int act, void* ws, void* stream);
 int icl_rstd_from_var(const float* var, float* rstd, int c, float eps, void* stream);
+int icl_norm_bwd_given_sums(const float* gy, const float* x, const float* mean, const float* rstd, const float* part, int nslots, float* gx,
+                            int n, int c, int64_t s, int act, void* stream);
 
 int icl_norm_finalize_stats(const float* part, int n, int c, int nslots, float eps, float* mean, float* rstd, float* ss, void* stream);
 int icl_norm_apply(const float* x, const float* ss, float* y, int n, int c, int64_t s, void* stream);
@@ -65,6 +67,9 @@
 int icl_maxpool2_bwd(const float* gy, const uint8_t* idx, float* gx, int64_t nc, int dout, int hout, int wout, int pool_depth, void* stream);
 int icl_maxpool2_bwd_add(const float* gy, const uint8_t* idx, const float* add, float* gx, int n, int c, int dout, int hout, int wout,
                          int pool_depth, int64_t add_bstride, void* stream);
+int icl_maxpool2_bwd_add_sums_slots(int dout, int hout, int wout);
+int icl_maxpool2_bwd_add_sums(const float* gy, const uint8_t* idx, const float* add, float* gx, const float* xraw, const float* mean,
+                              const float* rstd, float* part, int n, int c, int dout, int hout, int wout, int64_t add_bstride, void* stream);
 
 int icl_trilinear_fwd(const float* x, float* y, int n, int c, int di, int hi, int wi, int dout, int hout, int wout,
                       int64_t y_bstride, int align_corners, void* stream);
@@ -143,6 +148,9 @@
 int64_t icl_conv3d_cin1_wgrad_ws_bytes(int n, int d, int h);
 int icl_conv3d_cin1_wgrad(const float* x, const float* gy, float* gw, void* ws, int n, int cout, int d, int h, int wd, int64_t x_bstride,
                           int64_t gy_bstride, void* stream);
+int64_t icl_conv3d_cin1_norm_wgrad_ws_bytes(int n, int cout, int d, int h, int w);
+int icl_conv3d_cin1_norm_wgrad(const float* x, const float* gz, const float* y, const float* mean, const float* rstd, const float* sums,
+                               int nslots, float* gw, void* ws, int n, int cout, int d, int h, int wd, int64_t x_bstride, void* stream);
 int icl_col2im3(const float* g, float* dx, int n, int c, int d, int h, int w, void* stream);
 
 int icl_depth_to_space2(const float* yt, float* out, int n, int d, int h, int w, int cout, int64_t out_bstride, void* stream);
```

Result: no change. 202.1 volumes/s (-0.5%).
